# SAP/nested-hashing-psi

Measured on AMD Instinct MI355X. Metric: server PIE ciphertexts/sec, higher is better.
Workload: dtype u64

## Files before the change

### nested_hashing_psi_amd/csrc/kernels.hpp

```cpp
#pragma once
#include <hip/hip_runtime.h>

#include <atomic>
#include <vector>

#include "params.hpp"

namespace piehip {

struct PerDeviceOnce {
    std::atomic<unsigned long long> done{0};
    bool first_on_current_device()
    {
        int dev = 0;
        if (hipGetDevice(&dev) != hipSuccess || dev < 0 || dev > 63) return true;
        const unsigned long long bit = 1ULL << dev;
        return (done.fetch_or(bit) & bit) == 0;
    }
};

enum class NttKernel { radix2, blocked32, blocked16 };
struct NttRoute {
    NttKernel kernel;
    u32 s0;
    u32 global_stages;
    bool extra() const { return kernel != NttKernel::radix2 && !global_stages; }
};

struct NttPlan {
    const u64 *tables;
    const u64 *twp;
    const u64 *twc = nullptr;
    const u64 *twc_fold = nullptr;
    const u64 *twk16 = nullptr;
    const DevConsts *dc;
    u32 N, logN;
    u32 num_cus;
    u32 max_slots = 0;
    bool lane_order = false;
    bool fold = false;
    NttKernel lane_kernel = NttKernel::radix2;
    u32 lane_logn = 0;
    u32 lane_T = 0;
    u32 lane_kp = 16;
    bool small_moduli = false;
    bool xq_reuse = false;
    bool x_direct = false;
    bool fused_tensor = false;
    bool d01_eval_q = false;
    bool digits_with_d01 = false;
    bool digit_lift_lane = false;
    bool digit_lift_std = false;
    u32 transform_cus() const
    {
        if (!max_slots) return num_cus;
        const u32 c = (max_slots + 1) / 2;
        return c < num_cus ? (c ? c : 1u) : num_cus;
    }
};
void ntt_plan_decide(NttPlan &pl, bool lazy_ok, bool small_moduli);
NttRoute ntt_route(const NttPlan &pl, bool inverse, bool sigma, bool folded);

void build_twc_table(const u64 *nat_pairs, u32 logN, u32 s0, std::vector<u64> &out);
void build_twk16_table(const u64 *nat_pairs, u32 s0, u32 slice_log, std::vector<u64> &out);
void ntt_sigma_inverse_map(u32 logN, u32 s0, std::vector<u32> &map);
void ntt16_sigma_inverse_map(u32 logN, u32 s0, std::vector<u32> &map);
struct NttExtra {
    u64 *copy_out = nullptr;
    u32 copy_K = 1, copy_L = 1, copy_M = 1;
    u32 skip_L = 0, skip_M = 0;
    bool lazy_out = false;
    bool folded = false;
    bool x_lane_in = false;
};
void launch_ntt(const NttPlan &pl, u64 *data, u32 nlimbs, u32 mod_base, u32 mod_count, bool inverse, hipStream_t st,
                bool sigma = false, bool folded = false, const NttExtra *ex = nullptr);
void launch_ntt_fast(const NttPlan &pl, const u64 *twc, u32 s0, u64 *data, u32 nlimbs, u32 mod_base, u32 mod_count, bool inverse,
                     bool sigma, hipStream_t st, const u64 *lift_src = nullptr, u32 lift_L = 0, const NttExtra *ex = nullptr);
struct Ntt16Digits {
    const u64 *d2;
    size_t stride2;
    u64 *dig;
    u32 nb, L;
};
void launch_ntt16(const NttPlan &pl, u64 *data, u32 nlimbs, u32 mod_base, u32 mod_count, bool inverse, bool sigma, hipStream_t st,
                  const NttExtra *ex, const Ntt16Digits *dg = nullptr);
#ifndef PIEHIP_FUSE_TENSOR
#define PIEHIP_FUSE_TENSOR 1
#endif
#ifndef PIEHIP_D01_EVAL_Q
#define PIEHIP_D01_EVAL_Q 1
#endif
void launch_ntt16_tensor(const NttPlan &pl, const u64 *e, u64 *d, u32 nb, u32 M, hipStream_t st, u32 eval_q_L = 0);
void launch_ntt_digits(const NttPlan &pl, const u64 *d2, u64 *dig, u32 nb, u32 L, bool sigma, hipStream_t st);

struct StageAXOut {
    u64 *out = nullptr;
    u32 M = 0, logns = 0;
};
void launch_stage_a(const DevConsts *dc, u32 N, u32 L, u32 K, u32 b, u32 E, const u64 *idx, const u64 *minus,
                    const u64 *db, u64 *acc, hipStream_t st, bool small_moduli, u32 bstride = 0, u32 h0 = 0, u32 hn = 0, u32 nq = 1,
                    u32 q = 0, const StageAXOut *xo = nullptr);
static const u32 STAGE_A_MAX_QUERIES = 8;
struct StageAQueries {
    const u64 *idx[STAGE_A_MAX_QUERIES];
    const u64 *minus[STAGE_A_MAX_QUERIES];
};
void launch_stage_a_batch(const DevConsts *dc, u32 N, u32 L, u32 K, u32 b, u32 E, const StageAQueries &qs, u32 nq, const u64 *db,
                          u64 *acc, hipStream_t st, bool small_moduli, u32 bstride = 0, u32 h0 = 0, u32 hn = 0,
                          const StageAXOut *xo = nullptr);

void launch_expand_q_to_qp(const DevConsts *dc, u32 N, u32 L, const u64 *in, size_t in_stride_outer,
                           size_t in_stride_inner, u32 n_outer, u64 *out, u32 out_polys, u32 out_slot, hipStream_t st,
                           bool small_moduli, bool fold = false, bool skip_q = false);
void launch_scale_pq_expand(const DevConsts *dc, u32 N, u32 L, const u64 *in, size_t in_stride_outer,
                            size_t in_stride_inner, u32 n_outer, u64 *out, u32 out_polys, u32 out_slot, hipStream_t st,
                            bool small_moduli, bool fold = false);
void launch_expand_both(const DevConsts *dc, u32 N, u32 L, const u64 *x, size_t sx, const u64 *y, size_t sy, size_t si, u32 n_outer,
                        u64 *out, hipStream_t st, bool small_moduli, bool fold = false, bool skip_q = false);
void launch_tensor(const DevConsts *dc, u32 N, u32 M, const u64 *e, u64 *d, u32 nb, hipStream_t st, bool small_moduli);
void launch_scale_round(const DevConsts *dc, u32 N, u32 L, const u64 *d, u32 nb, u64 *out01, size_t stride01, u64 *out2,
                        size_t stride2, hipStream_t st, bool small_moduli, bool fold = false, bool fold_comp2 = false, bool p_only01 = false);
void launch_digits(const DevConsts *dc, u32 N, u32 L, const u64 *d2, size_t stride2, u32 nb, u64 *dig, hipStream_t st,
                   bool fold = false);
void launch_relin_mac(const DevConsts *dc, u32 N, u32 L, const u64 *d01, size_t stride01, const u64 *dig, const u64 *key,
                      const u64 *mask, u64 *out, u32 nb, hipStream_t st, bool small_moduli, const u32 *out_map = nullptr, size_t key_stride = 0,
                      u32 key_group = 1, u32 sigma_T = 0, u32 sigma_kp = 16, u32 mask_div = 1, const u64 *eqp = nullptr, u32 eqp_M = 0);
void launch_bcast_mul_plain(const DevConsts *dc, u32 N, u32 L, const u64 *x, size_t xs, u32 group, const u64 *pt, size_t ps_outer,
                            size_t ps_inner, u64 *out, u32 nct, hipStream_t st);
void launch_rot_prepare(const DevConsts *dc, u32 N, u32 L, const u64 *x, const u32 *maps, u32 map_group, bool acc, bool identity_first,
                        u64 *d01, u64 *d2, u32 nct, hipStream_t st);
void launch_sum_mul_plain(const DevConsts *dc, u32 N, u32 L, const u64 *x, u32 group, const u64 *pt, size_t pt_stride, u64 *out,
                          size_t out_stride, u32 ngroups, hipStream_t st);
void launch_host_flag(u64 *flag_dev, u64 value, hipStream_t st);
void launch_ct_add(const DevConsts *dc, u32 N, u32 L, const u64 *x, const u64 *y, u64 *out, u32 nct, hipStream_t st);
void launch_ct_mul_plain(const DevConsts *dc, u32 N, u32 L, const u64 *x, const u64 *pt, size_t pt_stride, u64 *out,
                         u32 nct, hipStream_t st, u32 pt_div = 1);
bool launch_limb_drop(const DevConsts *dc, u32 N, u32 L, u32 keep, const u64 *in, u64 *out, u32 npoly, hipStream_t st);
void launch_permute(u32 N, const u64 *in, const u32 *map, u64 *out, u32 nrows, hipStream_t st);
void launch_encode_scatter(const DevConsts *dc, u32 N, u32 M, const int64_t *slots, u32 B, const u32 *inv_pos, u64 *u,
                           u32 npt, hipStream_t st);
void launch_encode_lift(const DevConsts *dc, u32 N, u32 L, u32 M, const u64 *u, u64 *out, u32 npt, hipStream_t st, u32 l0 = 0);

void launch_stage_a_slice(const DevConsts *dc, u32 N, u32 L, u32 u_lo, u32 un, u32 b, u32 E, const StageAQueries &qs, u32 nq,
                          const u64 *db, u64 *acc, hipStream_t st, bool small_moduli);
void launch_place_accumulators(u32 N, u32 L, u32 K, u32 u_lo, u32 un, u32 bin_lo, u32 bn, u32 nq, const u64 *src, u64 *acc,
                               const StageAXOut *xo, hipStream_t st);

size_t hash_sort_temp_bytes(u32 n, u32 e);
hipError_t launch_hash_build(const u64 *d_tab, const u64 *d_items, u32 n, u32 k, u32 e, u32 K, u32 b, u32 E, u64 evict_seed,
                             u64 shuffle_seed, u64 *d_tbl, u32 *d_keys, u32 *d_vals, u32 *d_start, void *d_temp, size_t temp_bytes,
                             u32 *d_fail, hipStream_t st);
void launch_shuffle_rows(u64 *d_tbl, u32 rows, u32 b, u32 E, u64 seed, hipStream_t st);
void launch_gather_slots(const u64 *d_tbl, u32 B, u32 K, u32 b, u32 E, u64 t, int64_t *d_slots, u32 *d_fail, hipStream_t st);
void launch_mask_slots(u64 t, u32 b, u32 B, u64 seed, int64_t *d_out, hipStream_t st);

void launch_enc_message(const DevConsts *dc, u32 N, u32 L, u32 M, const u64 *coeff_t, const int32_t *e, u64 *em, u32 nct, hipStream_t st);
void launch_enc_finish(const DevConsts *dc, u32 N, u32 L, const u64 *em, const u64 *sk, const u64 *a_in, u64 *out, u32 nct,
                       hipStream_t st);
void launch_ks_finish(const DevConsts *dc, u32 N, u32 L, const u64 *e, const u64 *sk, const u64 *s_from, u64 *ks, hipStream_t st);
void launch_square(const DevConsts *dc, u32 N, u32 L, const u64 *s, u64 *s2, hipStream_t st);
void launch_dec_dot(const DevConsts *dc, u32 N, u32 L, const u64 *ct, const u64 *sk, u64 *xs, u32 nct, hipStream_t st);
void launch_dec_round(const DevConsts *dc, u32 N, u32 L, u32 M, const u64 *xs, u64 *coeff_t, u32 nct, hipStream_t st);
void launch_decode_gather(const DevConsts *dc, u32 N, u32 M, const u64 *u, const u32 *slot_pos, u32 B, int64_t *slots, u32 nct,
                          hipStream_t st);

struct SeedJob {
    u64 *dst;
    u32 seed[8];
};
static const u32 SEED_MAX_JOBS_PER_LAUNCH = 65535;
void launch_expand_uniform(const DevConsts *dc, u32 N, u32 L, const SeedJob *jobs, u32 njobs, hipStream_t st);

}
```

### nested_hashing_psi_amd/csrc/kernels_ntt.hip

```cpp
#include "kernels.hpp"

#include <algorithm>
#include <cassert>

namespace piehip {

static const u32 NTT_LDS_MAX_LOG = 14;

struct NttArgs {
    u64 *data;
    const u64 *tables;
    const DevConsts *dc;
    u32 N, logN;
    u32 s0;
    u32 mod_base, mod_count;
};

template <bool INV>
__global__ void __launch_bounds__(1024) ntt_lds_generic(NttArgs a)
{
    extern __shared__ u64 s[];
    const u32 tid = threadIdx.x, nthr = blockDim.x;
    const u32 nl = a.N >> a.s0;
    const u32 limb = blockIdx.x >> a.s0, blk = blockIdx.x & ((1u << a.s0) - 1);
    const u32 mod = a.mod_base + limb % a.mod_count;
    const Mod m = a.dc->mod[mod];
    const u64 q = m.q, q2 = 2 * m.q;
    const u64 *tw = a.tables + (size_t)mod * 4 * a.N + (INV ? 2 * (size_t)a.N : 0);
    const u64 *tws = tw + a.N;
    u64 *g = a.data + (size_t)limb * a.N + (size_t)blk * nl;

    for (u32 i = tid; i < nl; i += nthr) s[i] = g[i];
    __syncthreads();

    if (!INV) {
        u32 logt = a.logN - a.s0 - 1;
        for (u32 ml = 1; ml < nl; ml <<= 1, logt--) {
            const u32 t = 1u << logt;
            for (u32 bi = tid; bi < nl / 2; bi += nthr) {
                const u32 i = bi >> logt, j = bi & (t - 1);
                const u32 x = (i << (logt + 1)) + j;
                const u32 k = (ml << a.s0) + blk * ml + i;
                const u64 w = tw[k], ws = tws[k];
                u64 u = s[x];
                u = u >= q2 ? u - q2 : u;
                const u64 v = mul_shoup_lazy(s[x + t], w, ws, q);
                s[x] = u + v;
                s[x + t] = u - v + q2;
            }
            __syncthreads();
        }
        for (u32 i = tid; i < nl; i += nthr) {
            u64 v = s[i];
            v = v >= q2 ? v - q2 : v;
            g[i] = v >= q ? v - q : v;
        }
    } else {
        u32 logt = 0;
        for (u32 hl = nl >> 1; hl >= 1; hl >>= 1, logt++) {
            const u32 t = 1u << logt;
            for (u32 bi = tid; bi < nl / 2; bi += nthr) {
                const u32 i = bi >> logt, j = bi & (t - 1);
                const u32 x = (i << (logt + 1)) + j;
                const u32 k = (hl << a.s0) + blk * hl + i;
                const u64 w = tw[k], ws = tws[k];
                const u64 u = s[x], v = s[x + t];
                const u64 sm = u + v;
                s[x] = sm >= q2 ? sm - q2 : sm;
                s[x + t] = mul_shoup_lazy(u - v + q2, w, ws, q);
            }
            __syncthreads();
        }
        if (a.s0 == 0) {
            for (u32 i = tid; i < nl; i += nthr) g[i] = mul_shoup(s[i], m.n_inv, m.n_inv_sh, q);
        } else {
            for (u32 i = tid; i < nl; i += nthr) {
                u64 v = s[i];
                g[i] = v >= q ? v - q : v;
            }
        }
    }
}

template <bool INV>
__global__ void __launch_bounds__(256) ntt_global_stage(NttArgs a, u32 mstage, u32 last_inverse)
{
    const u32 half = a.N >> 1;
    const u32 bi = blockIdx.x * 256 + threadIdx.x;
    const u32 limb = blockIdx.y;
    if (bi >= half) return;
    const u32 mod = a.mod_base + limb % a.mod_count;
    const Mod m = a.dc->mod[mod];
    const u64 q = m.q;
    const u64 *tw = a.tables + (size_t)mod * 4 * a.N + (INV ? 2 * (size_t)a.N : 0);
    const u64 *tws = tw + a.N;
    u32 logm = 0;
    while ((1u << logm) < mstage) logm++;
    const u32 logt = a.logN - 1 - logm, t = 1u << logt;
    const u32 i = bi >> logt, j = bi & (t - 1);
    const size_t x = (size_t)limb * a.N + ((size_t)i << (logt + 1)) + j;
    const u64 w = tw[mstage + i], ws = tws[mstage + i];
    const u64 u = a.data[x], v = a.data[x + t];
    if (!INV) {
        const u64 p = mul_shoup(v, w, ws, q);
        a.data[x] = addmod(u, p, q);
        a.data[x + t] = submod(u, p, q);
    } else {
        u64 sm = addmod(u, v, q);
        u64 df = mul_shoup(submod(u, v, q), w, ws, q);
        if (last_inverse) {
            sm = mul_shoup(sm, m.n_inv, m.n_inv_sh, q);
            df = mul_shoup(df, m.n_inv, m.n_inv_sh, q);
        }
        a.data[x] = sm;
        a.data[x + t] = df;
    }
}

static PerDeviceOnce g_attr_set[2];

NttRoute ntt_route(const NttPlan &pl, bool inverse, bool sigma, bool folded)
{
    assert((!sigma || pl.lane_order) && (!folded || pl.fold));
    const u32 s0 = pl.logN > NTT_LDS_MAX_LOG ? pl.logN - NTT_LDS_MAX_LOG : 0;
    if (!pl.lane_order) return {NttKernel::radix2, s0, s0};
    if (pl.lane_kernel == NttKernel::blocked16 && folded == pl.fold && (inverse || sigma)) return {NttKernel::blocked16, folded ? 1u : 0u, 0};
    if (folded) return {NttKernel::blocked32, 1, 0};
    return {NttKernel::blocked32, s0, s0};
}

void ntt_plan_decide(NttPlan &pl, bool lazy_ok, bool small_moduli)
{
    pl.lane_order = lazy_ok && pl.logN >= 12;
    pl.small_moduli = small_moduli;
    if (!pl.lane_order) return;
    const bool k16 = pl.logN >= 13 && pl.logN <= 15;
    pl.lane_kernel = k16 ? NttKernel::blocked16 : NttKernel::blocked32;
    pl.fold = pl.logN == 14 || pl.logN == 15;
    pl.lane_logn = pl.logN - ntt_route(pl, true, true, pl.fold).s0;
    pl.lane_T = (1u << pl.lane_logn) / (k16 ? 16 : 32);
    pl.lane_kp = k16 ? 8 : 16;
    pl.xq_reuse = ntt_route(pl, true, false, pl.fold).extra();
    pl.fused_tensor = PIEHIP_FUSE_TENSOR && k16 && small_moduli;
    pl.d01_eval_q = PIEHIP_D01_EVAL_Q && pl.fused_tensor;
    pl.digits_with_d01 = k16 && small_moduli;
    pl.x_direct = pl.xq_reuse && k16 && small_moduli;
    const NttRoute std_fwd = ntt_route(pl, false, false, false);
    pl.digit_lift_std = std_fwd.kernel == NttKernel::blocked32 && std_fwd.s0 == 0;
    pl.digit_lift_lane = pl.digit_lift_std && !k16;
}

void launch_ntt_digits(const NttPlan &pl, const u64 *d2, u64 *dig, u32 nb, u32 L, bool sigma, hipStream_t st)
{
    assert(sigma ? pl.digit_lift_lane : pl.digit_lift_std);
    launch_ntt_fast(pl, pl.twc, 0, dig, nb * L * L, 0, L, false, sigma, st, d2, L);
}

void launch_ntt(const NttPlan &pl, u64 *data, u32 nlimbs, u32 mod_base, u32 mod_count, bool inverse, hipStream_t st, bool sigma,
                bool folded, const NttExtra *ex)
{
    if (!nlimbs) return;
    const NttRoute r = ntt_route(pl, inverse, sigma, folded);
    if (r.kernel == NttKernel::blocked16) {
        launch_ntt16(pl, data, nlimbs, mod_base, mod_count, inverse, sigma, st, ex);
        return;
    }
    if (folded) {
        NttExtra exf;
        if (ex) exf = *ex;
        exf.folded = true;
        launch_ntt_fast(pl, pl.twc_fold, 1, data, nlimbs, mod_base, mod_count, inverse, sigma, st, nullptr, 0, &exf);
        return;
    }
    NttArgs a;
    a.data = data;
    a.tables = pl.tables;
    a.dc = pl.dc;
    a.N = pl.N;
    a.logN = pl.logN;
    a.s0 = r.s0;
    a.mod_base = mod_base;
    a.mod_count = mod_count;
    const u32 nl = pl.N >> a.s0;
    const size_t lds = (size_t)nl * sizeof(u64);
    const u32 threads = std::min(std::max(nl / 2, 64u), 1024u);
    const bool radix2 = r.kernel == NttKernel::radix2;
    if (radix2 && g_attr_set[inverse ? 1 : 0].first_on_current_device())
        (void)hipFuncSetAttribute(inverse ? (const void *)ntt_lds_generic<true> : (const void *)ntt_lds_generic<false>,
                                  hipFuncAttributeMaxDynamicSharedMemorySize, (1 << NTT_LDS_MAX_LOG) * 8);
    const dim3 ggrid((pl.N / 2 + 255) / 256, nlimbs);
    if (!inverse) {
        for (u32 ms = 1; ms < (1u << r.global_stages); ms <<= 1)
            hipLaunchKernelGGL(ntt_global_stage<false>, ggrid, dim3(256), 0, st, a, ms, 0u);
        if (radix2) hipLaunchKernelGGL(ntt_lds_generic<false>, dim3(nlimbs << a.s0), dim3(threads), lds, st, a);
    } else if (radix2) {
        hipLaunchKernelGGL(ntt_lds_generic<true>, dim3(nlimbs << a.s0), dim3(threads), lds, st, a);
    }
    if (!radix2) launch_ntt_fast(pl, pl.twc, r.s0, data, nlimbs, mod_base, mod_count, inverse, sigma, st, nullptr, 0, ex);
    if (inverse)
        for (u32 ms = (1u << r.global_stages) >> 1; ms >= 1; ms >>= 1)
            hipLaunchKernelGGL(ntt_global_stage<true>, ggrid, dim3(256), 0, st, a, ms, ms == 1 ? 1u : 0u);
}

}
```

### nested_hashing_psi_amd/csrc/kernels_pie.hip

```cpp
#include <stdlib.h>

#include <cassert>

#include <algorithm>

#include "kernels.hpp"
#include "madasm.h"
#include "stage_a_common.h"

namespace piehip {

static const u32 TPB = 256;

typedef u64 u64x2 __attribute__((ext_vector_type(2)));


template <int BPT>
__global__ void __launch_bounds__(TPB) stage_a_kernel(const DevConsts *__restrict__ dc, u32 N, u32 L, u32 K, u32 b, u32 E,
                                                      const u64 *__restrict__ idx, const u64 *__restrict__ minus,
                                                      const u64 *__restrict__ db, u64 *__restrict__ acc, u32 bstride, u32 h0,
                                                      u32 nq, u32 q)
{
    const u32 n = 2 * (blockIdx.x * TPB + threadIdx.x);
    const u32 l = blockIdx.y;
    const u32 groups = b / BPT;
    const u32 h = h0 + blockIdx.z / groups, beta0 = (blockIdx.z % groups) * BPT;
    if (n >= N) return;
    const Mod m = dc->mod[l];
    const size_t LN = (size_t)L * N;
    const u64 *pi = idx + ((size_t)h * E) * 2 * LN + (size_t)l * N + n;
    const u64 *pd = db + (((size_t)h * bstride + beta0) * E) * LN + (size_t)l * N + n;
    const size_t bin_stride = (size_t)E * LN;
    U128 a[BPT][2][2];
#pragma unroll
    for (int t = 0; t < BPT; t++)
#pragma unroll
        for (int c = 0; c < 2; c++) a[t][c][0] = a[t][c][1] = U128{0, 0};
    for (u32 j = 0; j < E; j++) {
        const u64x2 i0 = *reinterpret_cast<const u64x2 *>(pi + (size_t)j * 2 * LN);
        const u64x2 i1 = *reinterpret_cast<const u64x2 *>(pi + (size_t)j * 2 * LN + LN);
        u64x2 d[BPT];
#pragma unroll
        for (int t = 0; t < BPT; t++) {
            typedef u64 u64v2 __attribute__((ext_vector_type(2)));
            const u64v2 v = __builtin_nontemporal_load(reinterpret_cast<const u64v2 *>(pd + (size_t)t * bin_stride + (size_t)j * LN));
            d[t].x = v.x, d[t].y = v.y;
        }
#pragma unroll
        for (int t = 0; t < BPT; t++) {
            mac128(a[t][0][0], i0.x, d[t].x);
            mac128(a[t][0][1], i0.y, d[t].y);
            mac128(a[t][1][0], i1.x, d[t].x);
            mac128(a[t][1][1], i1.y, d[t].y);
        }
        if ((j & 31) == 31) {
#pragma unroll
            for (int t = 0; t < BPT; t++)
#pragma unroll
                for (int c = 0; c < 2; c++)
#pragma unroll
                    for (int e = 0; e < 2; e++) a[t][c][e] = U128{reduce128(a[t][c][e], m), 0};
        }
    }
    const u64x2 m0 = *reinterpret_cast<const u64x2 *>(minus + (size_t)l * N + n);
    const u64x2 m1 = *reinterpret_cast<const u64x2 *>(minus + LN + (size_t)l * N + n);
#pragma unroll
    for (int t = 0; t < BPT; t++) {
        u64 *po = acc + ((((size_t)(beta0 + t) * nq + q) * K + h) * 2) * LN + (size_t)l * N + n;
        u64x2 r0, r1;
        r0.x = addmod(reduce128(a[t][0][0], m), m0.x, m.q);
        r0.y = addmod(reduce128(a[t][0][1], m), m0.y, m.q);
        r1.x = addmod(reduce128(a[t][1][0], m), m1.x, m.q);
        r1.y = addmod(reduce128(a[t][1][1], m), m1.y, m.q);
        *reinterpret_cast<u64x2 *>(po) = r0;
        *reinterpret_cast<u64x2 *>(po + LN) = r1;
    }
}

static const int SA_DEPTH = 4;
template <int BPT>
__global__ void __launch_bounds__(TPB) stage_a_mad_kernel(const DevConsts *__restrict__ dc, u32 N, u32 L, u32 K, u32 b, u32 E,
                                                          const u64 *__restrict__ idx, const u64 *__restrict__ minus,
                                                          const u64 *__restrict__ db, u64 *__restrict__ acc, u32 bstride, u32 h0,
                                                          u32 nq, u32 q, StageAXOut xo)
{
    const u32 nl = threadIdx.x;
    const u32 n = blockIdx.x * TPB + nl;
    const u32 l = blockIdx.y;
    const u32 groups = b / BPT;
    const u32 h = h0 + blockIdx.z / groups, beta0 = (blockIdx.z % groups) * BPT;
    if (n >= N) return;
    const Mod m = dc->mod[l];
    const size_t LN = (size_t)L * N;
    const u64 *pi = idx + ((size_t)h * E) * 2 * LN + (size_t)l * N + blockIdx.x * TPB;
    const u64 *pd = db + (((size_t)h * bstride + beta0) * E) * LN + (size_t)l * N + blockIdx.x * TPB;
    const size_t bin_stride = (size_t)E * LN;
    ColAcc a[BPT][2];
#pragma unroll
    for (int t = 0; t < BPT; t++) a[t][0] = a[t][1] = ColAcc{0, 0, 0};
    auto load_term = [&](u32 j, u64 (&vi)[2], u64 (&vd)[BPT]) {
        const u64 *pij = pi + (size_t)j * 2 * LN, *pdj = pd + (size_t)j * LN;
        vi[0] = pij[nl];
        vi[1] = (pij + LN)[nl];
#pragma unroll
        for (int t = 0; t < BPT; t++) vd[t] = __builtin_nontemporal_load(pdj + (size_t)t * bin_stride + nl);
    };
    u64 qiv[SA_DEPTH][2], qdv[SA_DEPTH][BPT];
#pragma unroll
    for (int d = 0; d < SA_DEPTH; d++)
        if ((u32)d < E) load_term(d, qiv[d], qdv[d]);
    auto term = [&](u32 j, u64 (&vi)[2], u64 (&vd)[BPT]) {
        const Split30 i0 = split30(vi[0]), i1 = split30(vi[1]);
#pragma unroll
        for (int t = 0; t < BPT; t++) colacc_mac2(a[t][0], a[t][1], i0, i1, vd[t]);
        if (j + SA_DEPTH < E) load_term(j + SA_DEPTH, vi, vd);
        if ((j % COLACC_MAX_TERMS) == COLACC_MAX_TERMS - 1 && j + 1 < E) {
#pragma unroll
            for (int t = 0; t < BPT; t++) colacc_carry(a[t][0]), colacc_carry(a[t][1]);
        }
        if ((j % COLACC_MAX_TOTAL) == COLACC_MAX_TOTAL - 1 && j + 1 < E) {
#pragma unroll
            for (int t = 0; t < BPT; t++)
#pragma unroll
                for (int c = 0; c < 2; c++) {
                    const u64 r = reduce124(colacc_value(a[t][c]), m);
                    a[t][c] = ColAcc{r & 0x3FFFFFFFull, r >> 30, 0};
                }
        }
    };
    for (u32 j = 0; j < E; j += SA_DEPTH) {
#pragma unroll
        for (int d = 0; d < SA_DEPTH; d++)
            if (j + d < E) term(j + d, qiv[d], qdv[d]);
    }
    const bool xdir = h == 0 && xo.out != nullptr;
    const u32 noff = n + ((xdir ? ~0u : 0u) & (lane_home(n, xo.logns) - n));
#pragma unroll
    for (int t = 0; t < BPT; t++) {
        const size_t row = (size_t)(beta0 + t) * nq + q;
        u64 *const base = xdir ? xo.out + ((row * 4) * xo.M + l) * N : acc + ((row * K + h) * 2) * LN + (size_t)l * N;
        const size_t cstride = xdir ? (size_t)xo.M * N : LN;
        u64 *const po = base + noff;
#pragma unroll
        for (int c = 0; c < 2; c++)
            po[(size_t)c * cstride] = addmod_nb(colacc_reduce<true>(a[t][c], m, 0 - m.q), minus[(size_t)c * LN + (size_t)l * N + n], m.q);
    }
}

template <int BPT, int Q, int DEPTH>
__global__ void __launch_bounds__(TPB) stage_a_mad_batch_kernel(const DevConsts *__restrict__ dc, u32 N, u32 L, u32 K, u32 b, u32 E,
                                                                StageAQueries qs, const u64 *__restrict__ db, u64 *__restrict__ acc,
                                                                u32 bstride, u32 h0, u32 nq, u32 q0, u32 tiles, StageAXOut xo)
{
    StageATile tl;
    if (!stage_a_tile((N + TPB - 1) / TPB, L, tiles, (b + BPT - 1) / BPT, tl)) return;
    const u32 nl = threadIdx.x, n0 = tl.bx * TPB, l = tl.l, h = h0 + tl.hz, beta0 = tl.grp * BPT;
    const u32 n = n0 + nl;
    if (n >= N) return;
    const u32 tmax = __builtin_amdgcn_readfirstlane(min((u32)BPT, b - beta0) - 1);
    const Mod m = dc->mod[l];
    const size_t LN = (size_t)L * N;
    const size_t ioff = ((size_t)h * E) * 2 * LN + (size_t)l * N + n0;
    const u64 *pd = db + (((size_t)h * bstride + beta0) * E) * LN + (size_t)l * N + n0;
    const size_t bin_stride = (size_t)E * LN;
    ColAcc a[Q][BPT][2];
#pragma unroll
    for (int q = 0; q < Q; q++)
#pragma unroll
        for (int t = 0; t < BPT; t++) a[q][t][0] = a[q][t][1] = ColAcc{0, 0, 0};
    auto load_term = [&](u32 j, u64 (&vi)[Q][2], u64 (&vd)[BPT]) {
#pragma unroll
        for (int q = 0; q < Q; q++) {
            const u64 *pij = qs.idx[q] + ioff + (size_t)j * 2 * LN;
            vi[q][0] = pij[nl];
            vi[q][1] = (pij + LN)[nl];
        }
        const u64 *pdj = pd + (size_t)j * LN;
#pragma unroll
        for (int t = 0; t < BPT; t++) vd[t] = __builtin_nontemporal_load(pdj + (size_t)min((u32)t, tmax) * bin_stride + nl);
    };
    u64 qiv[DEPTH][Q][2], qdv[DEPTH][BPT];
#pragma unroll
    for (int d = 0; d < DEPTH; d++)
        if ((u32)d < E) load_term(d, qiv[d], qdv[d]);
    auto term = [&](u32 j, u64 (&vi)[Q][2], u64 (&vd)[BPT]) {
#pragma unroll
        for (int q = 0; q < Q; q++) {
            const Split30 i0 = split30(vi[q][0]), i1 = split30(vi[q][1]);
#pragma unroll
            for (int t = 0; t < BPT; t++) colacc_mac2(a[q][t][0], a[q][t][1], i0, i1, vd[t]);
        }
        if (j + DEPTH < E) load_term(j + DEPTH, vi, vd);
        if ((j % COLACC_MAX_TERMS) == COLACC_MAX_TERMS - 1 && j + 1 < E) {
#pragma unroll
            for (int q = 0; q < Q; q++)
#pragma unroll
                for (int t = 0; t < BPT; t++) colacc_carry(a[q][t][0]), colacc_carry(a[q][t][1]);
        }
        if ((j % COLACC_MAX_TOTAL) == COLACC_MAX_TOTAL - 1 && j + 1 < E) {
#pragma unroll
            for (int q = 0; q < Q; q++)
#pragma unroll
                for (int t = 0; t < BPT; t++)
#pragma unroll
                    for (int c = 0; c < 2; c++) {
                        const u64 r = colacc_reduce<true>(a[q][t][c], m, 0 - m.q);
                        a[q][t][c] = ColAcc{r & 0x3FFFFFFFull, r >> 30, 0};
                    }
        }
    };
    for (u32 j = 0; j < E; j += DEPTH) {
#pragma unroll
        for (int d = 0; d < DEPTH; d++)
            if (j + d < E) term(j + d, qiv[d], qdv[d]);
    }
    const bool xdir = h == 0 && xo.out != nullptr;
    const u32 noff = n + ((xdir ? ~0u : 0u) & (lane_home(n, xo.logns) - n));
#pragma unroll
    for (int q = 0; q < Q; q++) {
        u64 mi[2];
#pragma unroll
        for (int c = 0; c < 2; c++) mi[c] = qs.minus[q][(size_t)c * LN + (size_t)l * N + n];
#pragma unroll
        for (int t = 0; t < BPT; t++) {
            if ((u32)t > tmax) continue;
            const size_t row = (size_t)(beta0 + t) * nq + q0 + q;
            u64 *const base = xdir ? xo.out + ((row * 4) * xo.M + l) * N : acc + ((row * K + h) * 2) * LN + (size_t)l * N;
            const size_t cstride = xdir ? (size_t)xo.M * N : LN;
            u64 *const po = base + noff;
#pragma unroll
            for (int c = 0; c < 2; c++) po[(size_t)c * cstride] = addmod_nb(colacc_reduce<true>(a[q][t][c], m, 0 - m.q), mi[c], m.q);
        }
    }
}

static void launch_stage_a_uniform(const DevConsts *dc, u32 N, u32 L, u32 K, u32 b, u32 E, const u64 *idx, const u64 *minus,
                                   const u64 *db, u64 *acc, hipStream_t st, bool mad, u32 bstride, u32 h0, u32 hn, int bpt, u32 nq,
                                   u32 q, StageAXOut xo)
{
    const int cpt = mad ? 1 : 2;
    dim3 grid((N / cpt + TPB - 1) / TPB, L, hn * (b / bpt));
#define SA(B_)                                                                                                       \
    do {                                                                                                             \
        if (mad) hipLaunchKernelGGL(stage_a_mad_kernel<B_>, grid, dim3(TPB), 0, st, dc, N, L, K, b, E, idx, minus, db, acc, bstride, h0, nq, q, xo); \
        else hipLaunchKernelGGL(stage_a_kernel<B_>, grid, dim3(TPB), 0, st, dc, N, L, K, b, E, idx, minus, db, acc, bstride, h0, nq, q);  \
    } while (0)
    switch (bpt) {
        case 8: hipLaunchKernelGGL(stage_a_kernel<8>, grid, dim3(TPB), 0, st, dc, N, L, K, b, E, idx, minus, db, acc, bstride, h0, nq, q); break;
        case 7: SA(7); break;
        case 6: SA(6); break;
        case 5: SA(5); break;
        case 4: SA(4); break;
        case 3: SA(3); break;
        case 2: SA(2); break;
        default: SA(1); break;
    }
#undef SA
}

void launch_stage_a(const DevConsts *dc, u32 N, u32 L, u32 K, u32 b, u32 E, const u64 *idx, const u64 *minus,
                    const u64 *db, u64 *acc, hipStream_t st, bool small_moduli, u32 bstride, u32 h0, u32 hn, u32 nq, u32 q,
                    const StageAXOut *xop)
{
    StageAXOut xo;
    if (xop && small_moduli) xo = *xop;
    if (!bstride) bstride = b;
    if (!hn) hn = K - h0;
    if (!nq) nq = 1;
    const bool mad = small_moduli;
    const u32 cap = mad ? 7 : 8;
    u32 bpt = 0;
    for (u32 c = cap; c >= 4; c--)
        if (b % c == 0) {
            bpt = c;
            break;
        }
    if (b <= cap) bpt = b;
    const size_t LN = (size_t)L * N;
    if (bpt) {
        launch_stage_a_uniform(dc, N, L, K, b, E, idx, minus, db, acc, st, mad, bstride, h0, hn, (int)bpt, nq, q, xo);
        return;
    }
    const u32 full = (b / cap) * cap, rest = b - full;
    launch_stage_a_uniform(dc, N, L, K, full, E, idx, minus, db, acc, st, mad, bstride, h0, hn, (int)cap, nq, q, xo);
    StageAXOut xr = xo;
    if (xr.out) xr.out += (size_t)full * nq * 4 * xr.M * N;
    launch_stage_a_uniform(dc, N, L, K, rest, E, idx, minus, db + (size_t)full * E * LN, acc + (size_t)full * nq * K * 2 * LN, st, mad,
                           bstride, h0, hn, (int)rest, nq, q, xr);
}

template <int Q, int BPT>
static void launch_stage_a_batch_qb(const DevConsts *dc, u32 N, u32 L, u32 K, u32 nb, u32 E, const StageAQueries &qs, const u64 *db,
                                    u64 *acc, hipStream_t st, u32 bstride, u32 h0, u32 hn, u32 nq, u32 q0, StageAXOut xo)
{
    const u32 nx = (N + TPB - 1) / TPB;
    constexpr int DEPTH = (Q == 4 || Q * BPT >= 9) ? 2 : 3;
    hipLaunchKernelGGL((stage_a_mad_batch_kernel<BPT, Q, DEPTH>), stage_a_grid(nx, L, hn, (nb + BPT - 1) / BPT), dim3(TPB), 0, st, dc, N, L, K,
                       nb, E, qs, db, acc, bstride, h0, nq, q0, nx * L * hn, xo);
}
template <int Q>
static void launch_stage_a_batch_q(const DevConsts *dc, u32 N, u32 L, u32 K, u32 b, u32 E, const StageAQueries &qs, const u64 *db,
                                   u64 *acc, hipStream_t st, u32 bstride, u32 h0, u32 hn, u32 nq, u32 q0, StageAXOut xo)
{
    constexpr u32 cap = Q == 2 ? 4 : 3;
    u32 bpt = 1, best = ~0u;
    for (u32 g = 1; g <= cap && g <= b; g++) {
        const u32 loads = ((b + g - 1) / g) * (2 * Q + g);
        if (loads <= best) best = loads, bpt = g;
    }
    if constexpr (cap >= 4)
        if (bpt == 4) return launch_stage_a_batch_qb<Q, 4>(dc, N, L, K, b, E, qs, db, acc, st, bstride, h0, hn, nq, q0, xo);
    if constexpr (cap >= 3)
        if (bpt == 3) return launch_stage_a_batch_qb<Q, 3>(dc, N, L, K, b, E, qs, db, acc, st, bstride, h0, hn, nq, q0, xo);
    if (bpt == 2) return launch_stage_a_batch_qb<Q, 2>(dc, N, L, K, b, E, qs, db, acc, st, bstride, h0, hn, nq, q0, xo);
    return launch_stage_a_batch_qb<Q, 1>(dc, N, L, K, b, E, qs, db, acc, st, bstride, h0, hn, nq, q0, xo);
}
void launch_stage_a_batch(const DevConsts *dc, u32 N, u32 L, u32 K, u32 b, u32 E, const StageAQueries &qs, u32 nq, const u64 *db,
                          u64 *acc, hipStream_t st, bool small_moduli, u32 bstride, u32 h0, u32 hn, const StageAXOut *xop)
{
    StageAXOut xo;
    if (xop && small_moduli) xo = *xop;
    if (!bstride) bstride = b;
    if (!hn) hn = K - h0;
    u32 q0 = 0;
    while (small_moduli && nq - q0 >= 2) {
        const u32 left = nq - q0, g = left == 5 || left == 6 ? 3 : std::min(left, 4u);
        StageAQueries sub = {};
        for (u32 q = 0; q < g; q++) sub.idx[q] = qs.idx[q0 + q], sub.minus[q] = qs.minus[q0 + q];
        if (g == 2) launch_stage_a_batch_q<2>(dc, N, L, K, b, E, sub, db, acc, st, bstride, h0, hn, nq, q0, xo);
        else if (g == 3) launch_stage_a_batch_q<3>(dc, N, L, K, b, E, sub, db, acc, st, bstride, h0, hn, nq, q0, xo);
        else launch_stage_a_batch_q<4>(dc, N, L, K, b, E, sub, db, acc, st, bstride, h0, hn, nq, q0, xo);
        q0 += g;
    }
    for (; q0 < nq; q0++)
        launch_stage_a(dc, N, L, K, b, E, qs.idx[q0], qs.minus[q0], db, acc, st, small_moduli, bstride, h0, hn, nq, q0, xop);
}

#define PIE_ITER_FENCE() __builtin_amdgcn_sched_barrier(0)
typedef const __attribute__((address_space(4))) DevConsts *DcC;
__device__ __forceinline__ DcC dc_iter(const DevConsts *dc)
{
    u64 v = (u64)dc;
    asm volatile("" : "+s"(v));
    return (DcC)v;
}
__device__ __forceinline__ Mod ld_mod(DcC c, u32 i)
{
    Mod m;
    m.q = c->mod[i].q, m.r0 = c->mod[i].r0, m.r1 = c->mod[i].r1, m.n_inv = 0, m.n_inv_sh = 0;
    m.fconst = c->mod[i].fconst, m.fshift = c->mod[i].fshift, m.pad = 0;
    return m;
}

__device__ __forceinline__ u64 neg_u(u64 m)
{
    u64 n = 0 - m;
    asm("" : "+s"(n));
    return n;
}
__device__ __forceinline__ u64 sel_neg(u64 x, u64 t, u32 &mask)
{
    u32 lo, hi, k;
    asm("v_ashrrev_i32 %[k], 31, %[th]\n\t"
        "v_bfi_b32 %[lo], %[k], %[xl], %[tl]\n\t"
        "v_bfi_b32 %[hi], %[k], %[xh], %[th]"
        : [lo] "=&v"(lo), [hi] "=&v"(hi), [k] "=&v"(k)
        : [xl] "v"((u32)x), [xh] "v"((u32)(x >> 32)), [tl] "v"((u32)t), [th] "v"((u32)(t >> 32)));
    mask = k;
    return ((u64)hi << 32) | lo;
}
__device__ __forceinline__ u64 csub_u(u64 x, u64 negm)
{
    u32 k;
    return sel_neg(x, x + negm, k);
}
__device__ __forceinline__ u64 mul_shoup_lazy_u(u64 a, u64 w, u64 wsh, u64 q) { return a * w - mulhi(a, wsh) * q; }
__device__ __forceinline__ u64 mul_shoup_u(u64 a, u64 w, u64 wsh, u64 q, u64 negq) { return csub_u(mul_shoup_lazy_u(a, w, wsh, q), negq); }
__device__ __forceinline__ u64 fixfrac_u(u64 y, const Mod &m) { return mulhi(y << m.fshift, m.fconst) >> 3; }
__device__ __forceinline__ void divmod_shoup_u(u64 a, u64 w, u64 wsh, u64 q, u64 negq, u64 &quot, u64 &rem)
{
    const u64 qe = mulhi(a, wsh);
    const u64 r = a * w - qe * q;
    u32 k;
    rem = sel_neg(r, r + negq, k);
    quot = qe + 1 + (u64)(int64_t)(int32_t)k;
}
__device__ __forceinline__ u64 reduce123_u(U128 z, const Mod &m, u64 negq, u64 neg2q)
{
    const u64 mu = (m.r1 << 59) | (m.r0 >> 5);
    const u64 zh = (z.hi << 5) | (z.lo >> 59);
    const u64 qhat = mulhi(zh, mu);
    return csub_u(csub_u(z.lo - qhat * m.q, neg2q), negq);
}

#define PIE_SHOUP63_HEAD                                        \
    "v_mad_u64_u32 v[60:61], vcc, %[al], %[sh], 0\n\t"          \
    "v_mad_u64_u32 v[64:65], vcc, %[al], %[wl], 0\n\t"          \
    "v_mad_u64_u32 v[60:61], vcc, %[ah], %[sl], v[60:61]\n\t"   \
    "v_mad_u64_u32 v[66:67], vcc, %[al], %[wh], 0\n\t"          \
    "v_lshlrev_b32 v70, 1, %[ah]\n\t"                           \
    "v_mad_u64_u32 v[66:67], vcc, %[ah], %[wl], v[66:67]\n\t"   \
    "v_lshrrev_b64 v[60:61], 31, v[60:61]\n\t"                  \
    "v_mad_u64_u32 v[62:63], vcc, v70, %[sh], v[60:61]\n\t"     \
    "v_mad_u64_u32 v[66:67], vcc, v62, %[nqh], v[66:67]\n\t"    \
    "v_mad_u64_u32 v[66:67], vcc, v63, %[nql], v[66:67]\n\t"    \
    "v_add_u32 v65, v65, v66\n\t"
#define PIE_SHOUP63_IN(a, w, wsh, nq)                                                                                        \
    [al] "v"((u32)(a)), [ah] "v"((u32)((a) >> 32)), [wl] "s"((u32)(w)), [wh] "s"((u32)((w) >> 32)), [sl] "s"((u32)((wsh) >> 1)), \
        [sh] "s"((u32)((wsh) >> 33)), [nql] "s"((u32)(nq)), [nqh] "s"((u32)((nq) >> 32))
__device__ __forceinline__ u64 shoup63_lazy(u64 a, u64 w, u64 wsh, u64 nq)
{
    u64 r;
    asm(PIE_SHOUP63_HEAD
        "v_mad_u64_u32 %[r], vcc, v62, %[nql], v[64:65]"
        : [r] "=v"(r)
        : PIE_SHOUP63_IN(a, w, wsh, nq)
        : PIE_ASM_CLOB);
    return r;
}
__device__ __forceinline__ u64 shoup63(u64 a, u64 w, u64 wsh, u64 nq)
{
    u32 lo, hi;
    const u64 n2q = 2 * nq;
    asm(PIE_SHOUP63_HEAD
        "v_mad_u64_u32 v[64:65], vcc, v62, %[nql], v[64:65]\n\t"
        "v_lshl_add_u64 v[68:69], v[64:65], 0, %[n2q]\n\t"
        "v_ashrrev_i32 v71, 31, v69\n\t"
        "v_bfi_b32 v64, v71, v64, v68\n\t"
        "v_bfi_b32 v65, v71, v65, v69\n\t"
        "v_lshl_add_u64 v[68:69], v[64:65], 0, %[n1q]\n\t"
        "v_ashrrev_i32 v71, 31, v69\n\t"
        "v_bfi_b32 %[lo], v71, v64, v68\n\t"
        "v_bfi_b32 %[hi], v71, v65, v69"
        : [lo] "=v"(lo), [hi] "=v"(hi)
        : PIE_SHOUP63_IN(a, w, wsh, nq), [n2q] "s"(n2q), [n1q] "s"(nq)
        : PIE_ASM_CLOB);
    return ((u64)hi << 32) | lo;
}
__device__ __forceinline__ void divmod63(u64 a, u64 w, u64 wsh, u64 nq, u64 &quot, u64 &rem)
{
    u32 lo, hi;
    u64 qt;
    const u64 n2q = 2 * nq;
    asm(PIE_SHOUP63_HEAD
        "v_mad_u64_u32 v[64:65], vcc, v62, %[nql], v[64:65]\n\t"
        "v_lshl_add_u64 v[68:69], v[64:65], 0, %[n2q]\n\t"
        "v_ashrrev_i64 v[60:61], 63, v[68:69]\n\t"
        "v_bfi_b32 v64, v60, v64, v68\n\t"
        "v_bfi_b32 v65, v60, v65, v69\n\t"
        "v_lshl_add_u64 v[62:63], v[60:61], 1, v[62:63]\n\t"
        "v_lshl_add_u64 v[68:69], v[64:65], 0, %[n1q]\n\t"
        "v_ashrrev_i64 v[60:61], 63, v[68:69]\n\t"
        "v_bfi_b32 %[lo], v60, v64, v68\n\t"
        "v_bfi_b32 %[hi], v60, v65, v69\n\t"
        "v_lshl_add_u64 v[62:63], v[60:61], 0, v[62:63]\n\t"
        "v_lshl_add_u64 %[qt], v[62:63], 0, 3"
        : [lo] "=v"(lo), [hi] "=v"(hi), [qt] "=v"(qt)
        : PIE_SHOUP63_IN(a, w, wsh, nq), [n2q] "s"(n2q), [n1q] "s"(nq)
        : PIE_ASM_CLOB);
    quot = qt;
    rem = ((u64)hi << 32) | lo;
}
__device__ __forceinline__ u64 mulhi_sb(u64 a, u64 b)
{
    u64 r;
    asm("v_mul_hi_u32 v60, %[al], %[bl]\n\t"
        "v_mov_b32 v61, 0\n\t"
        "v_mad_u64_u32 v[62:63], vcc, %[al], %[bh], v[60:61]\n\t"
        "v_mad_u64_u32 v[62:63], vcc, %[ah], %[bl], v[62:63]\n\t"
        "v_mad_u64_u32 v[66:67], s[96:97], %[ah], %[bh], 0\n\t"
        "v_lshrrev_b64 v[64:65], 32, v[62:63]\n\t"
        "v_addc_co_u32 v65, vcc, 0, v65, vcc\n\t"
        "v_lshl_add_u64 %[r], v[66:67], 0, v[64:65]"
        : [r] "=v"(r)
        : [al] "v"((u32)a), [ah] "v"((u32)(a >> 32)), [bl] "s"((u32)b), [bh] "s"((u32)(b >> 32))
        : PIE_ASM_CLOB, "s96", "s97");
    return r;
}
__device__ __forceinline__ void colacc_mac_small(ColAcc &a, u32 v, u64 c)
{
    const Split30 s = split30(c);
    a.c0 = mad_u(v, s.lo, a.c0);
    a.c1 = mad_u(v, s.hi, a.c1);
}

template <bool ASM>
__device__ __forceinline__ u64 mshoup(u64 a, u64 w, u64 wsh, u64 q, u64 negq)
{
    return ASM ? shoup63(a, w, wsh, negq) : mul_shoup_u(a, w, wsh, q, negq);
}
template <bool ASM>
__device__ __forceinline__ void mdivmod(u64 a, u64 w, u64 wsh, u64 q, u64 negq, u64 &quot, u64 &rem)
{
    if (ASM)
        divmod63(a, w, wsh, negq, quot, rem);
    else
        divmod_shoup_u(a, w, wsh, q, negq, quot, rem);
}
template <bool ASM>
__device__ __forceinline__ u64 mfixfrac(u64 y, const Mod &m)
{
    return ASM ? (mulhi_sb(y << m.fshift, m.fconst) >> 3) : fixfrac_u(y, m);
}

template <u32 NS, bool MAD>
__device__ __forceinline__ U128 dot128(const u64 *y, const u64 (&c)[NS])
{
    if (MAD) {
        ColAcc a = {0, 0, 0};
#pragma unroll
        for (u32 i = 0; i < NS; i++) colacc_mac(a, split30(y[i]), split30(c[i]));
        return colacc_value(a);
    }
    U128 acc = {0, 0};
#pragma unroll
    for (u32 i = 0; i < NS; i++) mac128(acc, y[i], c[i]);
    return acc;
}

template <u32 NS, bool MAD, bool LZ = false>
__device__ __forceinline__ u64 crt_out(const u64 *y, const u64 (&hat)[NS], u64 v, u64 prodmod, const Mod &tm, u64 negq, u64 neg2q)
{
    if (MAD && NS <= 7) {
        ColAcc a = {0, 0, 0};
#pragma unroll
        for (u32 i = 0; i < NS; i++) colacc_mac(a, split30(y[i]), split30(hat[i]));
        colacc_mac_small(a, (u32)v, tm.q - prodmod);
        return LZ ? colacc_reduce123_lazy(a, tm, negq) : colacc_reduce<false>(a, tm, negq);
    }
    U128 acc = dot128<NS, MAD>(y, hat);
    mac128(acc, v, tm.q - prodmod);
    return reduce128(acc, tm);
}

__device__ __forceinline__ void fold_load(const DevConsts *dc, u32 a, u64 u, u64 v, u64 &x0, u64 &x1)
{
    PIE_ITER_FENCE();
    const DcC c = dc_iter(dc);
    const u64 q = c->mod[a].q, nq = neg_u(q);
    x0 = shoup63(u + v, c->fold_ia[a], c->fold_ia_sh[a], nq);
    x1 = shoup63(u + (4 * q - v), c->fold_ib[a], c->fold_ib_sh[a], nq);
}
__device__ __forceinline__ void fold_store(const DevConsts *dc, u32 a, u64 u, u64 v, u64 &y0, u64 &y1)
{
    const DcC c = dc_iter(dc);
    const u64 q = c->mod[a].q;
    const u64 t = shoup63_lazy(v, c->fold_w[a], c->fold_w_sh[a], neg_u(q));
    y0 = u + t;
    y1 = u + (4 * q - t);
}

template <u32 L, bool MAD, bool YIN, int NP, bool LZ = false>
__device__ __forceinline__ void expand_core(const DevConsts *dc, const u64 (&x)[NP][L], u64 (&out)[NP][2 * L + 1])
{
    constexpr u32 Lp = L + 1;
    u64 y[NP][L];
    u64 fsum[NP];
#pragma unroll
    for (int p = 0; p < NP; p++) fsum[p] = 0;
#pragma unroll
    for (u32 i = 0; i < L; i++) {
        PIE_ITER_FENCE();
        const DcC c = dc_iter(dc);
        const Mod mi = ld_mod(c, i);
        const u64 w = c->qhat_inv[i], wsh = c->qhat_inv_sh[i], nq = neg_u(mi.q);
#pragma unroll
        for (int p = 0; p < NP; p++) {
            out[p][i] = x[p][i];
            y[p][i] = YIN ? x[p][i] : mshoup<MAD>(x[p][i], w, wsh, mi.q, nq);
            fsum[p] += mfixfrac<MAD>(y[p][i], mi);
        }
    }
#pragma unroll
    for (u32 j = 0; j < Lp; j++) {
        PIE_ITER_FENCE();
        const DcC c = dc_iter(dc);
        const Mod pj = ld_mod(c, L + j);
        u64 hat[L];
#pragma unroll
        for (u32 i = 0; i < L; i++) hat[i] = c->qhat_modp[i][j];
        const u64 prodmod = c->Q_modp[j], nq = neg_u(pj.q), n2q = neg_u(2 * pj.q);
#pragma unroll
        for (int p = 0; p < NP; p++) out[p][L + j] = crt_out<L, MAD, LZ>(y[p], hat, (fsum[p] + FIX_HALF) >> 60, prodmod, pj, nq, n2q);
    }
}

template <u32 L, bool MAD, bool YIN, int NP, bool LZ = false>
__device__ __forceinline__ void scale_pq_core(const DevConsts *dc, const u64 (&x)[NP][L], u64 (&out)[NP][2 * L + 1])
{
    constexpr u32 Lp = L + 1;
    u64 y[NP][L];
    u64 fsum[NP];
    U128 itot[NP];
#pragma unroll
    for (int p = 0; p < NP; p++) fsum[p] = 0, itot[p] = U128{0, 0};
#pragma unroll
    for (u32 i = 0; i < L; i++) {
        PIE_ITER_FENCE();
        const DcC c = dc_iter(dc);
        const Mod mi = ld_mod(c, i);
        const u64 w = c->qhat_inv[i], wsh = c->qhat_inv_sh[i], pw = c->P_modq[i], pwsh = c->P_modq_sh[i], nq = neg_u(mi.q);
#pragma unroll
        for (int p = 0; p < NP; p++) {
            y[p][i] = YIN ? x[p][i] : mshoup<MAD>(x[p][i], w, wsh, mi.q, nq);
            u64 fl, z;
            mdivmod<MAD>(y[p][i], pw, pwsh, mi.q, nq, fl, z);
            add128(itot[p], U128{fl, 0});
            fsum[p] += mfixfrac<MAD>(z, mi);
        }
    }
    u64 yp[NP][Lp];
    u64 fs2[NP];
#pragma unroll
    for (int p = 0; p < NP; p++) {
        add128(itot[p], U128{(fsum[p] + FIX_HALF) >> 60, 0});
        fs2[p] = 0;
    }
#pragma unroll
    for (u32 j = 0; j < Lp; j++) {
        PIE_ITER_FENCE();
        const DcC c = dc_iter(dc);
        const Mod pj = ld_mod(c, L + j);
        u64 col[L];
#pragma unroll
        for (u32 i = 0; i < L; i++) col[i] = c->PI_modp[i][j];
        const u64 w = c->phat_inv[j], wsh = c->phat_inv_sh[j], nq = neg_u(pj.q);
#pragma unroll
        for (int p = 0; p < NP; p++) {
            u64 r;
            if (MAD) {
                ColAcc a = {itot[p].lo, 0, 0};
#pragma unroll
                for (u32 i = 0; i < L; i++) colacc_mac(a, split30(y[p][i]), split30(col[i]));
                r = LZ ? colacc_reduce123_lazy(a, pj, nq) : colacc_reduce<false>(a, pj, nq);
            } else {
                U128 acc = dot128<L, MAD>(y[p], col);
                add128(acc, itot[p]);
                r = reduce128(acc, pj);
            }
            out[p][L + j] = r;
            yp[p][j] = mshoup<MAD>(r, w, wsh, pj.q, nq);
            fs2[p] += mfixfrac<MAD>(yp[p][j], pj);
        }
    }
#pragma unroll
    for (u32 i = 0; i < L; i++) {
        PIE_ITER_FENCE();
        const DcC c = dc_iter(dc);
        const Mod mi = ld_mod(c, i);
        u64 hat[Lp];
#pragma unroll
        for (u32 j = 0; j < Lp; j++) hat[j] = c->phat_modq[j][i];
        const u64 prodmod = c->P_modq[i], nq = neg_u(mi.q), n2q = neg_u(2 * mi.q);
#pragma unroll
        for (int p = 0; p < NP; p++) out[p][i] = crt_out<Lp, MAD, LZ>(yp[p], hat, (fs2[p] + FIX_HALF) >> 60, prodmod, mi, nq, n2q);
    }
}

template <bool SCALE, bool FOLD, u32 L, bool MAD, bool SKIPQ>
__device__ __forceinline__ void expand_body(const DevConsts *__restrict__ dc, u32 N, const u64 *__restrict__ in, size_t so, size_t si,
                                            u64 *__restrict__ out, u32 out_polys, u32 out_slot, u32 by)
{
    constexpr bool YIN = FOLD && (SCALE || SKIPQ);
    const u32 n = blockIdx.x * TPB + threadIdx.x;
    const u32 H = N / 2;
    if (n >= (FOLD ? H : N)) return;
    const u32 o = by >> 1, c = by & 1;
    constexpr u32 M = 2 * L + 1;
    const u64 *pin = in + (size_t)o * so + (size_t)c * si + n;
    u64 *pout = out + ((size_t)(o * out_polys + out_slot + c) * M) * N + n;
    constexpr int NP = FOLD ? 2 : 1;
    u64 x[NP][L], y[NP][M];
#pragma unroll
    for (u32 i = 0; i < L; i++) {
        if (YIN) {
            PIE_ITER_FENCE();
            const DcC c = dc_iter(dc);
            const u64 q = c->mod[i].q, nq = neg_u(q), u = pin[(size_t)i * N], v = pin[(size_t)i * N + H];
            x[0][i] = shoup63(u + v, c->fold_iaq[i], c->fold_iaq_sh[i], nq);
            x[NP - 1][i] = shoup63(u + (4 * q - v), c->fold_ibq[i], c->fold_ibq_sh[i], nq);
        } else if (FOLD) {
            fold_load(dc, i, pin[(size_t)i * N], pin[(size_t)i * N + H], x[0][i], x[NP - 1][i]);
        } else {
            x[0][i] = pin[(size_t)i * N];
        }
    }
    constexpr bool LZ = FOLD && MAD;
    if (SCALE)
        scale_pq_core<L, MAD, YIN, NP, LZ>(dc, x, y);
    else
        expand_core<L, MAD, YIN, NP, LZ>(dc, x, y);
#pragma unroll
    for (u32 a = 0; a < M; a++) {
        if (!SCALE && a < L && SKIPQ) continue;
        PIE_ITER_FENCE();
        if (FOLD) {
            u64 y0, y1;
            fold_store(dc, a, y[0][a], y[NP - 1][a], y0, y1);
            pout[(size_t)a * N] = y0;
            pout[(size_t)a * N + H] = y1;
        } else {
            pout[(size_t)a * N] = y[0][a];
        }
    }
}

template <bool SCALE, bool FOLD, u32 L, bool MAD, bool SKIPQ>
__global__ void __launch_bounds__(TPB) expand_kernel(const DevConsts *__restrict__ dc, u32 N, const u64 *__restrict__ in,
                                                     size_t so, size_t si, u64 *__restrict__ out, u32 out_polys, u32 out_slot)
{
    expand_body<SCALE, FOLD, L, MAD, SKIPQ>(dc, N, in, so, si, out, out_polys, out_slot, blockIdx.y);
}
template <bool FOLD, u32 L, bool MAD, bool SKIPQ>
__global__ void __launch_bounds__(TPB) expand_both_kernel(const DevConsts *__restrict__ dc, u32 N, const u64 *__restrict__ x, size_t sx,
                                                          const u64 *__restrict__ y, size_t sy, size_t si, u64 *__restrict__ out,
                                                          u32 n_outer)
{
    if (blockIdx.y < 2 * n_outer)
        expand_body<true, FOLD, L, MAD, false>(dc, N, y, sy, si, out, 4, 2, blockIdx.y);
    else
        expand_body<false, FOLD, L, MAD, SKIPQ>(dc, N, x, sx, si, out, 4, 0, blockIdx.y - 2 * n_outer);
}
void launch_expand_both(const DevConsts *dc, u32 N, u32 L, const u64 *x, size_t sx, const u64 *y, size_t sy, size_t si, u32 n_outer,
                        u64 *out, hipStream_t st, bool small_moduli, bool fold, bool skip_q)
{
    dim3 grid(((fold ? N / 2 : N) + TPB - 1) / TPB, n_outer * 4);
#define EB(F_, L_, M_, Q_) hipLaunchKernelGGL((expand_both_kernel<F_, L_, M_, Q_>), grid, dim3(TPB), 0, st, dc, N, x, sx, y, sy, si, out, n_outer)
#define EBL(L_)                                                                          \
    case L_:                                                                             \
        if (fold && small_moduli) { if (skip_q) EB(true, L_, true, true); else EB(true, L_, true, false); }      \
        else if (fold) { if (skip_q) EB(true, L_, false, true); else EB(true, L_, false, false); }                 \
        else if (small_moduli) { if (skip_q) EB(false, L_, true, true); else EB(false, L_, true, false); }       \
        else { if (skip_q) EB(false, L_, false, true); else EB(false, L_, false, false); }                         \
        break;
    switch (L) { EBL(1) EBL(2) EBL(3) EBL(4) EBL(5) EBL(6) EBL(7) }
#undef EBL
#undef EB
}

static void launch_expand_common(bool scale, bool fold, const DevConsts *dc, u32 N, u32 L, const u64 *in, size_t so, size_t si,
                                 u32 n_outer, u64 *out, u32 out_polys, u32 out_slot, hipStream_t st, bool small_moduli, bool skip_q = false)
{
    dim3 grid(((fold ? N / 2 : N) + TPB - 1) / TPB, n_outer * 2);
#define EX(S_, F_, L_, Q_)                                                                                                    \
    do {                                                                                                                      \
        if (small_moduli)                                                                                                   \
            hipLaunchKernelGGL((expand_kernel<S_, F_, L_, true, Q_>), grid, dim3(TPB), 0, st, dc, N, in, so, si, out, out_polys, out_slot); \
        else                                                                                                                  \
            hipLaunchKernelGGL((expand_kernel<S_, F_, L_, false, Q_>), grid, dim3(TPB), 0, st, dc, N, in, so, si, out, out_polys, out_slot); \
    } while (0)
#define EXL(L_)                                                         \
    case L_:                                                            \
        if (scale) {                                                    \
            if (fold) EX(true, true, L_, false); else EX(true, false, L_, false); \
        } else if (skip_q) {                                            \
            if (fold) EX(false, true, L_, true); else EX(false, false, L_, true); \
        } else {                                                        \
            if (fold) EX(false, true, L_, false); else EX(false, false, L_, false); \
        }                                                               \
        break;
    switch (L) { EXL(1) EXL(2) EXL(3) EXL(4) EXL(5) EXL(6) EXL(7) }
#undef EXL
#undef EX
}
void launch_expand_q_to_qp(const DevConsts *dc, u32 N, u32 L, const u64 *in, size_t so, size_t si, u32 n_outer, u64 *out,
                           u32 out_polys, u32 out_slot, hipStream_t st, bool small_moduli, bool fold, bool skip_q)
{
    launch_expand_common(false, fold, dc, N, L, in, so, si, n_outer, out, out_polys, out_slot, st, small_moduli, skip_q);
}
void launch_scale_pq_expand(const DevConsts *dc, u32 N, u32 L, const u64 *in, size_t so, size_t si, u32 n_outer, u64 *out,
                            u32 out_polys, u32 out_slot, hipStream_t st, bool small_moduli, bool fold)
{
    launch_expand_common(true, fold, dc, N, L, in, so, si, n_outer, out, out_polys, out_slot, st, small_moduli);
}

template <bool MAD>
__global__ void __launch_bounds__(TPB) tensor_kernel(const DevConsts *dc, u32 N, u32 M, const u64 *__restrict__ e,
                                                     u64 *__restrict__ d)
{
    const u32 n = 2 * (blockIdx.x * TPB + threadIdx.x);
    if (n >= N) return;
    const u32 a = blockIdx.y, bin = blockIdx.z;
    const Mod m = dc->mod[a];
    const size_t MN = (size_t)M * N;
    const u64 *pe = e + (size_t)bin * 4 * MN + (size_t)a * N + n;
    u64 *pd = d + (size_t)bin * 3 * MN + (size_t)a * N + n;
    const u64x2 va0 = *reinterpret_cast<const u64x2 *>(pe), va1 = *reinterpret_cast<const u64x2 *>(pe + MN),
                vb0 = *reinterpret_cast<const u64x2 *>(pe + 2 * MN), vb1 = *reinterpret_cast<const u64x2 *>(pe + 3 * MN);
    u64x2 r0, r1, r2;
#pragma unroll
    for (int k = 0; k < 2; k++) {
        u64 a0 = k ? va0.y : va0.x, a1 = k ? va1.y : va1.x, b0 = k ? vb0.y : vb0.x, b1 = k ? vb1.y : vb1.x;
        u64 d0, d1, d2;
        if (MAD) {
            const u64 nq = neg_u(m.q), n2q = neg_u(2 * m.q), n4q = neg_u(4 * m.q);
            a0 = csub_u(csub_u(a0, n4q), n2q), a1 = csub_u(csub_u(a1, n4q), n2q);
            b0 = csub_u(csub_u(b0, n4q), n2q), b1 = csub_u(csub_u(b1, n4q), n2q);
            const Split30 sa0 = split30(a0), sa1 = split30(a1), sb0 = split30(b0), sb1 = split30(b1);
            ColAcc c = {0, 0, 0};
            colacc_mac(c, sa0, sb0);
            d0 = colacc_reduce<false>(c, m, nq);
            c = ColAcc{0, 0, 0};
            colacc_mac(c, sa0, sb1);
            colacc_mac(c, sa1, sb0);
            d1 = colacc_reduce<false>(c, m, nq);
            c = ColAcc{0, 0, 0};
            colacc_mac(c, sa1, sb1);
            d2 = colacc_reduce<false>(c, m, nq);
        } else {
            d0 = mulmod(a0, b0, m);
            U128 x = mul128(a0, b1);
            mac128(x, a1, b0);
            d1 = reduce128(x, m);
            d2 = mulmod(a1, b1, m);
        }
        if (k) r0.y = d0, r1.y = d1, r2.y = d2;
        else r0.x = d0, r1.x = d1, r2.x = d2;
    }
    *reinterpret_cast<u64x2 *>(pd) = r0;
    *reinterpret_cast<u64x2 *>(pd + MN) = r1;
    *reinterpret_cast<u64x2 *>(pd + 2 * MN) = r2;
}
void launch_tensor(const DevConsts *dc, u32 N, u32 M, const u64 *e, u64 *d, u32 nb, hipStream_t st, bool small_moduli)
{
    dim3 grid((N / 2 + TPB - 1) / TPB, M, nb);
    if (small_moduli)
        hipLaunchKernelGGL(tensor_kernel<true>, grid, dim3(TPB), 0, st, dc, N, M, e, d);
    else
        hipLaunchKernelGGL(tensor_kernel<false>, grid, dim3(TPB), 0, st, dc, N, M, e, d);
}

template <u32 L, bool MAD, int NP, bool PRE = false, bool PONLY = false>
__device__ __forceinline__ void scale_round_core(const DevConsts *dc, const u64 (&d)[NP][2 * L + 1], u64 (&out)[NP][L], bool lz = false)
{
    constexpr u32 Lp = L + 1;
    u64 yp[NP][Lp];
    u64 fsum[NP];
    U128 itot[NP];
#pragma unroll
    for (int p = 0; p < NP; p++) fsum[p] = 0, itot[p] = U128{0, 0};
#pragma unroll
    for (u32 j = 0; j < Lp; j++) {
        PIE_ITER_FENCE();
        const DcC c = dc_iter(dc);
        const Mod pj = ld_mod(c, L + j);
        const u64 w = c->qp_hat_inv[L + j], wsh = c->qp_hat_inv_sh[L + j], tw = c->tQ_modp[j], twsh = c->tQ_modp_sh[j], nq = neg_u(pj.q);
#pragma unroll
        for (int p = 0; p < NP; p++) {
            yp[p][j] = PRE ? d[p][L + j] : mshoup<MAD>(d[p][L + j], w, wsh, pj.q, nq);
            u64 fl, z;
            mdivmod<MAD>(yp[p][j], tw, twsh, pj.q, nq, fl, z);
            add128(itot[p], U128{fl, 0});
            fsum[p] += mfixfrac<MAD>(z, pj);
        }
    }
#pragma unroll
    for (int p = 0; p < NP; p++) add128(itot[p], U128{(fsum[p] + FIX_HALF) >> 60, 0});
#pragma unroll
    for (u32 k = 0; k < L; k++) {
        PIE_ITER_FENCE();
        const DcC c = dc_iter(dc);
        const Mod qk = ld_mod(c, k);
        u64 col[Lp];
#pragma unroll
        for (u32 j = 0; j < Lp; j++) col[j] = c->tQF_modq[j][k];
        const u64 tp = c->tPinv_modq[k], nq = neg_u(qk.q);
#pragma unroll
        for (int p = 0; p < NP; p++) {
            if (MAD && L <= 6) {
                ColAcc a = {itot[p].lo, 0, 0};
#pragma unroll
                for (u32 j = 0; j < Lp; j++) colacc_mac(a, split30(yp[p][j]), split30(col[j]));
                if (PONLY)
                    ;
                else if (PRE)
                    a.c0 += d[p][k];
                else
                    colacc_mac(a, split30(d[p][k]), split30(tp));
                out[p][k] = (L <= 5 && lz) ? colacc_reduce123_lazy(a, qk, nq) : colacc_reduce<(L > 5)>(a, qk, nq);
            } else {
                U128 acc = dot128<Lp, MAD>(yp[p], col);
                if (PONLY)
                    ;
                else if (PRE)
                    add128(acc, U128{d[p][k], 0});
                else
                    mac128(acc, d[p][k], tp);
                add128(acc, itot[p]);
                out[p][k] = reduce128(acc, qk);
            }
        }
    }
}

template <bool FOLD, u32 L, bool MAD, bool PONLY>
__device__ __forceinline__ void scale_round_comp(const DevConsts *__restrict__ dc, u32 N, u32 n, const u64 *__restrict__ pin,
                                                 u64 *__restrict__ pout, bool fold_out, bool lz)
{
    const u32 H = N / 2;
    constexpr u32 M = 2 * L + 1;
    constexpr int NP = FOLD ? 2 : 1;
    u64 x[NP][M], y[NP][L];
#pragma unroll
    for (u32 a = PONLY ? L : 0; a < M; a++) {
        if (FOLD) {
            PIE_ITER_FENCE();
            const DcC c = dc_iter(dc);
            const u32 ak = a < L ? a : 0, aj = a < L ? 0 : a - L;
            const u64 q = c->mod[a].q, nq = neg_u(q), u = pin[(size_t)a * N], v = pin[(size_t)a * N + H];
            const u64 wa = a < L ? c->fold_iat[ak] : c->fold_iap[aj], was = a < L ? c->fold_iat_sh[ak] : c->fold_iap_sh[aj];
            const u64 wb = a < L ? c->fold_ibt[ak] : c->fold_ibp[aj], wbs = a < L ? c->fold_ibt_sh[ak] : c->fold_ibp_sh[aj];
            x[0][a] = shoup63(u + v, wa, was, nq);
            x[NP - 1][a] = shoup63(u + (4 * q - v), wb, wbs, nq);
        } else {
            x[0][a] = pin[(size_t)a * N];
        }
    }
    scale_round_core<L, MAD, NP, FOLD, PONLY>(dc, x, y, lz);
#pragma unroll
    for (u32 k = 0; k < L; k++) {
        PIE_ITER_FENCE();
        if (FOLD) {
            u64 y0 = y[0][k], y1 = y[NP - 1][k];
            if (fold_out) fold_store(dc, k, y[0][k], y[NP - 1][k], y0, y1);
            pout[(size_t)k * N] = y0;
            pout[(size_t)k * N + H] = y1;
        } else {
            pout[(size_t)k * N] = y[0][k];
        }
    }
}
template <bool FOLD, u32 L, bool MAD, bool P01 = false>
__global__ void __launch_bounds__(TPB) scale_round_kernel(const DevConsts *__restrict__ dc, u32 N, const u64 *__restrict__ d,
                                                          u64 *__restrict__ out01, size_t stride01,
                                                          u64 *__restrict__ out2, size_t stride2, u32 fold_comp2)
{
    const u32 n = blockIdx.x * TPB + threadIdx.x;
    if (n >= (FOLD ? N / 2 : N)) return;
    const u32 comp = blockIdx.y, bin = blockIdx.z;
    constexpr u32 M = 2 * L + 1;
    const u64 *pin = d + ((size_t)(bin * 3 + comp) * M) * N + n;
    u64 *pout = comp < 2 ? out01 + (size_t)bin * stride01 + (size_t)comp * L * N + n : out2 + (size_t)bin * stride2 + n;
    const bool lz = FOLD && MAD && comp < 2 && !fold_comp2;
    if (P01 && comp < 2)
        scale_round_comp<FOLD, L, MAD, true>(dc, N, n, pin, pout, true, lz);
    else
        scale_round_comp<FOLD, L, MAD, false>(dc, N, n, pin, pout, comp < 2 || fold_comp2, lz);
}
void launch_scale_round(const DevConsts *dc, u32 N, u32 L, const u64 *d, u32 nb, u64 *out01, size_t stride01, u64 *out2,
                        size_t stride2, hipStream_t st, bool small_moduli, bool fold, bool fold_comp2, bool p_only01)
{
    assert(!p_only01 || (small_moduli && !fold_comp2));
    dim3 grid(((fold ? N / 2 : N) + TPB - 1) / TPB, 3, nb);
#define SRK(F_, L_, M_, P_) \
    hipLaunchKernelGGL((scale_round_kernel<F_, L_, M_, P_>), grid, dim3(TPB), 0, st, dc, N, d, out01, stride01, out2, stride2, (fold_comp2 && F_) ? 1u : 0u)
#define SRL(L_)                                                                        \
    case L_:                                                                           \
        if (p_only01) {                                                                \
            if (fold) SRK(true, L_, true, true); else SRK(false, L_, true, true);      \
        } else if (small_moduli) {                                                     \
            if (fold) SRK(true, L_, true, false); else SRK(false, L_, true, false);    \
        } else {                                                                       \
            if (fold) SRK(true, L_, false, false); else SRK(false, L_, false, false);  \
        }                                                                              \
        break;
    switch (L) { SRL(1) SRL(2) SRL(3) SRL(4) SRL(5) SRL(6) SRL(7) }
#undef SRK
#undef SRL
}

__device__ __forceinline__ u64 digit_lift(const DevConsts *dc, u32 i, u32 j, u64 v)
{
    const Mod &mj = dc->mod[j];
    const u64 qi = dc->mod[i].q;
    u64 r = (qi < 2 * mj.q) ? (v >= mj.q ? v - mj.q : v) : barrett128(0, v, mj);
    if (v > qi / 2) r = submod(r, dc->qi_modqj[i][j], mj.q);
    return r;
}
template <bool FOLD>
__global__ void __launch_bounds__(TPB) digits_kernel(const DevConsts *__restrict__ dc, u32 N, u32 L, const u64 *__restrict__ d2,
                                                     size_t stride2, u64 *__restrict__ dig)
{
    const u32 n = blockIdx.x * TPB + threadIdx.x;
    const u32 H = N / 2;
    if (n >= (FOLD ? H : N)) return;
    const u32 i = blockIdx.y / L, j = blockIdx.y % L, bin = blockIdx.z;
    const u64 *pin = d2 + (size_t)bin * stride2 + (size_t)i * N + n;
    u64 *pout = dig + (((size_t)bin * L + i) * L + j) * N + n;
    if (FOLD) {
        u64 y0, y1;
        fold_store(dc, j, digit_lift(dc, i, j, pin[0]), digit_lift(dc, i, j, pin[H]), y0, y1);
        pout[0] = y0;
        pout[H] = y1;
    } else {
        pout[0] = digit_lift(dc, i, j, pin[0]);
    }
}
void launch_digits(const DevConsts *dc, u32 N, u32 L, const u64 *d2, size_t stride2, u32 nb, u64 *dig, hipStream_t st, bool fold)
{
    dim3 grid(((fold ? N / 2 : N) + TPB - 1) / TPB, L * L, nb);
    if (fold)
        hipLaunchKernelGGL(digits_kernel<true>, grid, dim3(TPB), 0, st, dc, N, L, d2, stride2, dig);
    else
        hipLaunchKernelGGL(digits_kernel<false>, grid, dim3(TPB), 0, st, dc, N, L, d2, stride2, dig);
}

template <bool MAD, int KP, int RPT = 1, bool EQ = false>
__global__ void __launch_bounds__(TPB) relin_mac_kernel(const DevConsts *__restrict__ dc, u32 N, u32 L, const u64 *__restrict__ d01,
                                                        size_t stride01, const u64 *__restrict__ dig,
                                                        const u64 *__restrict__ key0, const u64 *__restrict__ mask,
                                                        u64 *__restrict__ out, const u32 *__restrict__ out_map,
                                                        size_t key_stride, u32 key_group, u32 T, u32 mask_div, u32 nb,
                                                        const u64 *__restrict__ eqp, u32 eqp_M)
{
    static_assert(RPT == 1 || MAD, "two rows per thread: the column-accumulator path");
    static_assert(!EQ || MAD, "the own-limb term: the column-accumulator path");
    constexpr bool TILE = KP > 0;
    constexpr u32 TT = TILE ? TPB / (KP ? KP : 1) : 1;
    __shared__ u64x2 s_tile[TILE ? 2 * RPT : 1][TILE ? TPB : 1];
    u32 n = 2 * (blockIdx.x * TPB + threadIdx.x);
    u32 std_pair = 0;
    if (TILE) {
        const u32 tiles = T / TT, slice = blockIdx.x / tiles, tau0 = (blockIdx.x % tiles) * TT;
        const u32 k = threadIdx.x / TT, tt = threadIdx.x % TT;
        n = 2 * (slice * KP * T + k * T + tau0 + tt);
        std_pair = slice * KP * T + KP * tau0;
    }
    if (n >= N) return;
    const u32 j = blockIdx.y;
    u32 rows[RPT];
    bool has[RPT];
    if (RPT == 1) {
        rows[0] = blockIdx.z, has[0] = true;
    } else {
        const u32 k = blockIdx.z / key_group, q = blockIdx.z % key_group;
        rows[0] = 2 * k * key_group + q, has[0] = rows[0] < nb;
        rows[RPT - 1] = rows[0] + key_group, has[RPT - 1] = rows[RPT - 1] < nb;
        if (!has[0]) return;
    }
    const u32 bin = rows[0];
    const u64 *key = key0 + (size_t)(bin % key_group) * key_stride;
    const Mod m = dc->mod[j];
    const size_t LN = (size_t)L * N;
    const u32 po = TILE ? 0 : (out_map ? out_map[n] : n);
    u64x2 res[RPT][2];
    if (MAD) {
        ColAcc a[RPT][2][2];
#pragma unroll
        for (int r = 0; r < RPT; r++)
#pragma unroll
            for (int c = 0; c < 2; c++) a[r][c][0] = a[r][c][1] = ColAcc{0, 0, 0};
        for (u32 i = 0; i < L; i++) {
            const u64x2 k0 = *reinterpret_cast<const u64x2 *>(key + (((size_t)i * 2 + 0) * L + j) * N + n);
            const u64x2 k1 = *reinterpret_cast<const u64x2 *>(key + (((size_t)i * 2 + 1) * L + j) * N + n);
            const Split30 k0x = split30(k0.x), k0y = split30(k0.y), k1x = split30(k1.x), k1y = split30(k1.y);
#pragma unroll
            for (int r = 0; r < RPT; r++) {
                if (r && !has[r]) continue;
                const u64x2 d = *reinterpret_cast<const u64x2 *>(dig + (((size_t)rows[r] * L + i) * L + j) * N + n);
                const Split30 dx = split30(d.x), dy = split30(d.y);
                colacc_mac(a[r][0][0], dx, k0x);
                colacc_mac(a[r][0][1], dy, k0y);
                colacc_mac(a[r][1][0], dx, k1x);
                colacc_mac(a[r][1][1], dy, k1y);
            }
        }
        const u64 nq = 0 - m.q;
        if (EQ) {
            const u64 n2q = neg_u(2 * m.q), n4q = neg_u(4 * m.q);
            const u64 tp = dc->tPinv_modq[j], tpsh = dc->tPinv_modq_sh[j];
            const size_t MN = (size_t)eqp_M * N;
#pragma unroll
            for (int r = 0; r < RPT; r++) {
                if (r && !has[r]) continue;
                const u64 *pe = eqp + (size_t)rows[r] * 4 * MN + (size_t)j * N + n;
                const u64x2 va0 = *reinterpret_cast<const u64x2 *>(pe), va1 = *reinterpret_cast<const u64x2 *>(pe + MN),
                            vb0 = *reinterpret_cast<const u64x2 *>(pe + 2 * MN), vb1 = *reinterpret_cast<const u64x2 *>(pe + 3 * MN);
#pragma unroll
                for (int k = 0; k < 2; k++) {
                    const Split30 sa0 = split30(csub_u(csub_u(k ? va0.y : va0.x, n4q), n2q)), sa1 = split30(csub_u(csub_u(k ? va1.y : va1.x, n4q), n2q));
                    const Split30 sb0 = split30(csub_u(csub_u(k ? vb0.y : vb0.x, n4q), n2q)), sb1 = split30(csub_u(csub_u(k ? vb1.y : vb1.x, n4q), n2q));
                    ColAcc t = {0, 0, 0};
                    colacc_mac(t, sa0, sb0);
                    const u64 v0 = shoup63_lazy(colacc_reduce123_lazy(t, m, nq), tp, tpsh, nq);
                    t = ColAcc{0, 0, 0};
                    colacc_mac(t, sa0, sb1);
                    colacc_mac(t, sa1, sb0);
                    const u64 v1 = shoup63_lazy(colacc_reduce123_lazy(t, m, nq), tp, tpsh, nq);
                    a[r][0][k].c0 += v0 & 0x3FFFFFFFull, a[r][0][k].c1 += v0 >> 30;
                    a[r][1][k].c0 += v1 & 0x3FFFFFFFull, a[r][1][k].c1 += v1 >> 30;
                }
            }
        }
#pragma unroll
        for (int r = 0; r < RPT; r++) {
            if (r && !has[r]) continue;
            u64x2 mk;
            if (mask) mk = *reinterpret_cast<const u64x2 *>(mask + (size_t)(rows[r] / mask_div) * LN + (size_t)j * N + n);
#pragma unroll
            for (int c = 0; c < 2; c++) {
                const u64x2 s = *reinterpret_cast<const u64x2 *>(d01 + (size_t)rows[r] * stride01 + (size_t)c * LN + (size_t)j * N + n);
                a[r][c][0].c0 += s.x;
                a[r][c][1].c0 += s.y;
                res[r][c].x = colacc_reduce<false>(a[r][c][0], m, nq);
                res[r][c].y = colacc_reduce<false>(a[r][c][1], m, nq);
                if (mask) {
                    ColAcc p0 = {0, 0, 0}, p1 = {0, 0, 0};
                    colacc_mac(p0, split30(res[r][c].x), split30(mk.x));
                    colacc_mac(p1, split30(res[r][c].y), split30(mk.y));
                    res[r][c].x = colacc_reduce<false>(p0, m, nq);
                    res[r][c].y = colacc_reduce<false>(p1, m, nq);
                }
            }
        }
    } else {
        u64x2 mk;
        if (mask) mk = *reinterpret_cast<const u64x2 *>(mask + (size_t)(bin / mask_div) * LN + (size_t)j * N + n);
        U128 acc[2][2];
#pragma unroll
        for (int c = 0; c < 2; c++)
#pragma unroll
            for (int e = 0; e < 2; e++) acc[c][e] = U128{0, 0};
        for (u32 i = 0; i < L; i++) {
            const u64x2 d = *reinterpret_cast<const u64x2 *>(dig + (((size_t)bin * L + i) * L + j) * N + n);
            const u64x2 k0 = *reinterpret_cast<const u64x2 *>(key + (((size_t)i * 2 + 0) * L + j) * N + n);
            const u64x2 k1 = *reinterpret_cast<const u64x2 *>(key + (((size_t)i * 2 + 1) * L + j) * N + n);
            mac128(acc[0][0], d.x, k0.x);
            mac128(acc[0][1], d.y, k0.y);
            mac128(acc[1][0], d.x, k1.x);
            mac128(acc[1][1], d.y, k1.y);
        }
#pragma unroll
        for (int c = 0; c < 2; c++) {
            const u64x2 s = *reinterpret_cast<const u64x2 *>(d01 + (size_t)bin * stride01 + (size_t)c * LN + (size_t)j * N + n);
            add128(acc[c][0], U128{s.x, 0});
            add128(acc[c][1], U128{s.y, 0});
            res[0][c].x = reduce128(acc[c][0], m);
            res[0][c].y = reduce128(acc[c][1], m);
            if (mask) {
                res[0][c].x = mulmod(res[0][c].x, mk.x, m);
                res[0][c].y = mulmod(res[0][c].y, mk.y, m);
            }
        }
    }
#pragma unroll
    for (int r = 0; r < RPT; r++)
#pragma unroll
        for (int c = 0; c < 2; c++) {
            if (r && !has[r]) continue;
            const u64x2 v = res[r][c];
            if (TILE)
                s_tile[2 * r + c][KP * (threadIdx.x % TT) + threadIdx.x / TT] = v;
            else
                *reinterpret_cast<u64x2 *>(out + ((size_t)rows[r] * 2 + c) * LN + (size_t)j * N + po) = v;
        }
    if (TILE) {
        __syncthreads();
#pragma unroll
        for (int r = 0; r < RPT; r++)
#pragma unroll
            for (int c = 0; c < 2; c++) {
                if (r && !has[r]) continue;
                *reinterpret_cast<u64x2 *>(out + ((size_t)rows[r] * 2 + c) * LN + (size_t)j * N + 2 * (std_pair + threadIdx.x)) = s_tile[2 * r + c][threadIdx.x];
            }
    }
}
void launch_relin_mac(const DevConsts *dc, u32 N, u32 L, const u64 *d01, size_t stride01, const u64 *dig, const u64 *key,
                      const u64 *mask, u64 *out, u32 nb, hipStream_t st, bool small_moduli, const u32 *out_map, size_t key_stride,
                      u32 key_group, u32 sigma_T, u32 sigma_kp, u32 mask_div, const u64 *eqp, u32 eqp_M)
{
    assert(!eqp || (small_moduli && eqp_M >= L));
    if (!key_group) key_group = 1;
    if (!mask_div) mask_div = 1;
    const bool tile = out_map && (sigma_kp == 16 || sigma_kp == 8) && sigma_T >= TPB / sigma_kp && sigma_T % (TPB / sigma_kp) == 0 &&
                      (N / 2) % TPB == 0;
    const int kp = tile ? (int)sigma_kp : 0;
    const bool two = small_moduli && nb >= 2 * key_group;
    const u32 zrows = two ? ((nb + 2 * key_group - 1) / (2 * key_group)) * key_group : nb;
    dim3 grid((N / 2 + TPB - 1) / TPB, L, zrows);
#define RME(M_, K_, R_, E_)                                                                                                            \
    hipLaunchKernelGGL((relin_mac_kernel<M_, K_, R_, E_>), grid, dim3(TPB), 0, st, dc, N, L, d01, stride01, dig, key, mask, out, out_map, \
                       key_stride, key_group, sigma_T, mask_div, nb, eqp, eqp_M)
#define RM(M_, K_, R_) RME(M_, K_, R_, false)
#define RQ(K_, R_) RME(true, K_, R_, true)
    if (eqp && two) {
        if (kp == 16) RQ(16, 2); else if (kp == 8) RQ(8, 2); else RQ(0, 2);
    } else if (eqp) {
        if (kp == 16) RQ(16, 1); else if (kp == 8) RQ(8, 1); else RQ(0, 1);
    } else if (two) {
        if (kp == 16) RM(true, 16, 2); else if (kp == 8) RM(true, 8, 2); else RM(true, 0, 2);
    } else if (small_moduli) {
        if (kp == 16) RM(true, 16, 1); else if (kp == 8) RM(true, 8, 1); else RM(true, 0, 1);
    } else {
        if (kp == 16) RM(false, 16, 1); else if (kp == 8) RM(false, 8, 1); else RM(false, 0, 1);
    }
#undef RQ
#undef RM
#undef RME
}

__global__ void host_flag_kernel(volatile u64 *flag, u64 value)
{
    *flag = value;
    __threadfence_system();
}
void launch_host_flag(u64 *flag_dev, u64 value, hipStream_t st)
{
    hipLaunchKernelGGL(host_flag_kernel, dim3(1), dim3(1), 0, st, (volatile u64 *)flag_dev, value);
}

__global__ void __launch_bounds__(TPB) ct_add_kernel(const DevConsts *dc, u32 N, u32 L, const u64 *__restrict__ x,
                                                     const u64 *__restrict__ y, u64 *__restrict__ out)
{
    const u32 n = blockIdx.x * TPB + threadIdx.x;
    if (n >= N) return;
    const u32 l = blockIdx.y % L;
    const size_t o = ((size_t)blockIdx.z * 2 * L + blockIdx.y) * N + n;
    out[o] = addmod(x[o], y[o], dc->mod[l].q);
}
void launch_ct_add(const DevConsts *dc, u32 N, u32 L, const u64 *x, const u64 *y, u64 *out, u32 nct, hipStream_t st)
{
    dim3 grid((N + TPB - 1) / TPB, 2 * L, nct);
    hipLaunchKernelGGL(ct_add_kernel, grid, dim3(TPB), 0, st, dc, N, L, x, y, out);
}
__global__ void __launch_bounds__(TPB) ct_mul_plain_kernel(const DevConsts *dc, u32 N, u32 L, const u64 *__restrict__ x,
                                                           const u64 *__restrict__ pt, size_t pt_stride,
                                                           u64 *__restrict__ out, u32 pt_div)
{
    const u32 n = blockIdx.x * TPB + threadIdx.x;
    if (n >= N) return;
    const u32 l = blockIdx.y % L;
    const size_t o = ((size_t)blockIdx.z * 2 * L + blockIdx.y) * N + n;
    out[o] = mulmod(x[o], pt[(size_t)(blockIdx.z / pt_div) * pt_stride + (size_t)l * N + n], dc->mod[l]);
}
void launch_ct_mul_plain(const DevConsts *dc, u32 N, u32 L, const u64 *x, const u64 *pt, size_t pt_stride, u64 *out,
                         u32 nct, hipStream_t st, u32 pt_div)
{
    dim3 grid((N + TPB - 1) / TPB, 2 * L, nct);
    hipLaunchKernelGGL(ct_mul_plain_kernel, grid, dim3(TPB), 0, st, dc, N, L, x, pt, pt_stride, out, pt_div ? pt_div : 1);
}

template <int L, int KEEP>
__global__ void __launch_bounds__(TPB) limb_drop_kernel(const DevConsts *__restrict__ dc, u32 N, u32 blocks_per_poly,
                                                        const u64 *__restrict__ in, u64 *__restrict__ out)
{
    const u32 poly = blockIdx.x / blocks_per_poly;
    const u32 n = (blockIdx.x % blocks_per_poly) * TPB + threadIdx.x;
    if (n >= N) return;
    const u64 *pin = in + (size_t)poly * L * N + n;
    u64 c[L];
#pragma unroll
    for (int i = 0; i < L; i++) c[i] = pin[(size_t)i * N];
#pragma unroll
    for (int l = L - 1; l >= KEEP; l--) {
        const u64 ql = dc->mod[l].q;
        const u64 v = c[l];
        const u64 s = (u64)((int64_t)((ql >> 1) - v) >> 63);
#pragma unroll
        for (int i = 0; i < l; i++) {
            const u64 off = dc->drop_off[l][i];
            const u64 x = c[i] - v + off + (s & (ql - off));
            c[i] = mul_shoup_u(x, dc->drop_inv[l][i], dc->drop_inv_sh[l][i], dc->mod[i].q, dc->drop_negq[i]);
        }
    }
    u64 *pout = out + (size_t)poly * KEEP * N + n;
#pragma unroll
    for (int i = 0; i < KEEP; i++) pout[(size_t)i * N] = c[i];
}
bool launch_limb_drop(const DevConsts *dc, u32 N, u32 L, u32 keep, const u64 *in, u64 *out, u32 npoly, hipStream_t st)
{
    if (keep < 1 || keep >= L || L > MAX_L || !npoly) return false;
    const u32 bpp = (N + TPB - 1) / TPB;
    const dim3 grid(bpp * npoly), block(TPB);
#define DROP_(L_, K_)                                                                                          \
    case (L_) * 8 + (K_):                                                                                      \
        hipLaunchKernelGGL((limb_drop_kernel<L_, K_>), grid, block, 0, st, dc, N, bpp, in, out);               \
        return true
    switch (L * 8 + keep) {
        DROP_(2, 1);
        DROP_(3, 1); DROP_(3, 2);
        DROP_(4, 1); DROP_(4, 2); DROP_(4, 3);
        DROP_(5, 1); DROP_(5, 2); DROP_(5, 3); DROP_(5, 4);
        DROP_(6, 1); DROP_(6, 2); DROP_(6, 3); DROP_(6, 4); DROP_(6, 5);
        DROP_(7, 1); DROP_(7, 2); DROP_(7, 3); DROP_(7, 4); DROP_(7, 5); DROP_(7, 6);
    }
#undef DROP_
    return false;
}

__global__ void __launch_bounds__(TPB) permute_kernel(u32 N, const u64 *__restrict__ in, const u32 *__restrict__ map,
                                                      u64 *__restrict__ out)
{
    const u32 p = blockIdx.x * TPB + threadIdx.x;
    if (p >= N) return;
    const size_t r = (size_t)blockIdx.y * N;
    out[r + p] = in[r + map[p]];
}
void launch_permute(u32 N, const u64 *in, const u32 *map, u64 *out, u32 nrows, hipStream_t st)
{
    dim3 grid((N + TPB - 1) / TPB, nrows);
    hipLaunchKernelGGL(permute_kernel, grid, dim3(TPB), 0, st, N, in, map, out);
}

__global__ void __launch_bounds__(TPB) bcast_mul_plain_kernel(const DevConsts *dc, u32 N, u32 L, const u64 *__restrict__ x,
                                                              size_t xs, u32 group, const u64 *__restrict__ pt, size_t ps_outer,
                                                              size_t ps_inner, u64 *__restrict__ out)
{
    const u32 n = blockIdx.x * TPB + threadIdx.x;
    if (n >= N) return;
    const u32 l = blockIdx.y % L, i = blockIdx.z, g = i / group, r = i % group;
    const size_t LN = (size_t)L * N;
    const size_t o = (size_t)blockIdx.y * N + n;
    out[(size_t)i * 2 * LN + o] = mulmod(x[(size_t)g * xs + o], pt[(size_t)g * ps_outer + (size_t)r * ps_inner + (size_t)l * N + n], dc->mod[l]);
}
void launch_bcast_mul_plain(const DevConsts *dc, u32 N, u32 L, const u64 *x, size_t xs, u32 group, const u64 *pt, size_t ps_outer,
                            size_t ps_inner, u64 *out, u32 nct, hipStream_t st)
{
    dim3 grid((N + TPB - 1) / TPB, 2 * L, nct);
    hipLaunchKernelGGL(bcast_mul_plain_kernel, grid, dim3(TPB), 0, st, dc, N, L, x, xs, group, pt, ps_outer, ps_inner, out);
}
__global__ void __launch_bounds__(TPB) rot_prepare_kernel(const DevConsts *dc, u32 N, u32 L, const u64 *__restrict__ x,
                                                          const u32 *__restrict__ maps, u32 map_group, u32 acc, u32 identity_first,
                                                          u64 *__restrict__ d01, u64 *__restrict__ d2)
{
    const u32 p = blockIdx.x * TPB + threadIdx.x;
    if (p >= N) return;
    const u32 l = blockIdx.y, i = blockIdx.z, r = i % map_group;
    const size_t LN = (size_t)L * N;
    const u64 *c0 = x + (size_t)i * 2 * LN + (size_t)l * N, *c1 = c0 + LN;
    u64 *o0 = d01 + (size_t)i * 2 * LN + (size_t)l * N, *o1 = o0 + LN, *o2 = d2 + (size_t)i * LN + (size_t)l * N;
    if (identity_first && r == 0) {
        o0[p] = c0[p];
        o1[p] = c1[p];
        o2[p] = 0;
        return;
    }
    const u32 s = maps[(size_t)r * N + p];
    const u64 q = dc->mod[l].q;
    o0[p] = acc ? addmod(c0[p], c0[s], q) : c0[s];
    o1[p] = acc ? c1[p] : 0;
    o2[p] = c1[s];
}
void launch_rot_prepare(const DevConsts *dc, u32 N, u32 L, const u64 *x, const u32 *maps, u32 map_group, bool acc, bool identity_first,
                        u64 *d01, u64 *d2, u32 nct, hipStream_t st)
{
    dim3 grid((N + TPB - 1) / TPB, L, nct);
    hipLaunchKernelGGL(rot_prepare_kernel, grid, dim3(TPB), 0, st, dc, N, L, x, maps, map_group ? map_group : 1u, acc ? 1u : 0u,
                       identity_first ? 1u : 0u, d01, d2);
}
__global__ void __launch_bounds__(TPB) sum_mul_plain_kernel(const DevConsts *dc, u32 N, u32 L, const u64 *__restrict__ x, u32 group,
                                                            const u64 *__restrict__ pt, size_t pt_stride, u64 *__restrict__ out,
                                                            size_t out_stride)
{
    const u32 n = blockIdx.x * TPB + threadIdx.x;
    if (n >= N) return;
    const u32 l = blockIdx.y % L, g = blockIdx.z;
    const size_t LN = (size_t)L * N;
    const size_t o = (size_t)blockIdx.y * N + n;
    const Mod m = dc->mod[l];
    u64 s = 0;
    for (u32 r = 0; r < group; r++) s = addmod(s, x[((size_t)g * group + r) * 2 * LN + o], m.q);
    out[(size_t)g * out_stride + o] = mulmod(s, pt[(size_t)g * pt_stride + (size_t)l * N + n], m);
}
void launch_sum_mul_plain(const DevConsts *dc, u32 N, u32 L, const u64 *x, u32 group, const u64 *pt, size_t pt_stride, u64 *out,
                          size_t out_stride, u32 ngroups, hipStream_t st)
{
    dim3 grid((N + TPB - 1) / TPB, 2 * L, ngroups);
    hipLaunchKernelGGL(sum_mul_plain_kernel, grid, dim3(TPB), 0, st, dc, N, L, x, group, pt, pt_stride, out, out_stride);
}

__global__ void __launch_bounds__(TPB) encode_scatter_kernel(const DevConsts *dc, u32 N, u32 M,
                                                             const int64_t *__restrict__ slots, u32 B,
                                                             const u32 *__restrict__ inv_pos, u64 *__restrict__ u)
{
    const u32 p = blockIdx.x * TPB + threadIdx.x;
    if (p >= N) return;
    const u64 t = dc->mod[M].q;
    const u32 s = inv_pos[p];
    u64 val = 0;
    if (s < B) {
        const int64_t v = slots[(size_t)blockIdx.y * B + s];
        const u64 mag = v < 0 ? (u64)(-v) : (u64)v;
        val = v < 0 ? (mag ? t - mag : 0) : mag;
    }
    u[(size_t)blockIdx.y * N + p] = val;
}
void launch_encode_scatter(const DevConsts *dc, u32 N, u32 M, const int64_t *slots, u32 B, const u32 *inv_pos, u64 *u,
                           u32 npt, hipStream_t st)
{
    dim3 grid((N + TPB - 1) / TPB, npt);
    hipLaunchKernelGGL(encode_scatter_kernel, grid, dim3(TPB), 0, st, dc, N, M, slots, B, inv_pos, u);
}
__global__ void __launch_bounds__(TPB) encode_lift_kernel(const DevConsts *dc, u32 N, u32 L, u32 M,
                                                          const u64 *__restrict__ u, u64 *__restrict__ out, u32 l0)
{
    const u32 n = blockIdx.x * TPB + threadIdx.x;
    if (n >= N) return;
    const u64 t = dc->mod[M].q;
    const u64 v = u[(size_t)blockIdx.z * N + n];
    const u64 q = dc->mod[l0 + blockIdx.y].q;
    out[((size_t)blockIdx.z * L + blockIdx.y) * N + n] = v > t / 2 ? q - (t - v) : v;
}
void launch_encode_lift(const DevConsts *dc, u32 N, u32 L, u32 M, const u64 *u, u64 *out, u32 npt, hipStream_t st, u32 l0)
{
    dim3 grid((N + TPB - 1) / TPB, L, npt);
    hipLaunchKernelGGL(encode_lift_kernel, grid, dim3(TPB), 0, st, dc, N, L, M, u, out, l0);
}

}
```

### nested_hashing_psi_amd/csrc/params.cpp

```cpp
#include "params.hpp"

#include <string.h>

namespace piehip {

typedef unsigned __int128 u128;

static inline u64 mm(u64 a, u64 b, u64 q) { return (u64)(((u128)a * b) % q); }

u64 powmod(u64 a, u64 e, u64 q)
{
    u64 r = 1 % q;
    a %= q;
    for (; e; e >>= 1) {
        if (e & 1) r = mm(r, a, q);
        a = mm(a, a, q);
    }
    return r;
}
u64 invmod(u64 a, u64 q) { return powmod(a % q, q - 2, q); }

u32 bitrev32(u32 x, u32 bits)
{
    u32 r = 0;
    for (u32 i = 0; i < bits; i++, x >>= 1) r = (r << 1) | (x & 1);
    return r;
}

bool is_prime_u64(u64 n)
{
    static const u64 B[] = {2, 3, 5, 7, 11, 13, 17, 19, 23, 29, 31, 37};
    if (n < 2) return false;
    for (u64 b : B) {
        if (n == b) return true;
        if (n % b == 0) return false;
    }
    u64 d = n - 1;
    int s = 0;
    for (; !(d & 1); d >>= 1) s++;
    for (u64 b : B) {
        u64 x = powmod(b, d, n);
        if (x == 1 || x == n - 1) continue;
        bool witness = true;
        for (int r = 1; r < s && witness; r++) {
            x = mm(x, x, n);
            if (x == n - 1) witness = false;
        }
        if (witness) return false;
    }
    return true;
}

bool prime_chain(u32 N, u64 below, u32 count, u64 *out)
{
    const u64 step = 2ULL * N;
    if (below <= step + 1) return false;
    u64 c = ((below - 2) / step) * step + 1;
    u32 got = 0;
    for (; got < count && c > step; c -= step)
        if (is_prime_u64(c)) out[got++] = c;
    return got == count;
}

u64 min_primitive_root(u64 q, u32 N)
{
    const u64 m = 2ULL * N;
    if ((q - 1) % m) return 0;
    u64 root = 0;
    for (u64 g = 2; g < 1000 && !root; g++) {
        u64 x = powmod(g, (q - 1) / m, q);
        if (powmod(x, N, q) == q - 1) root = x;
    }
    if (!root) return 0;
    const u64 sq = mm(root, root, q);
    u64 cur = root, best = root;
    for (u32 k = 1; k < N; k++) {
        cur = mm(cur, sq, q);
        if (cur < best) best = cur;
    }
    return best;
}

static inline u64 shoup(u64 w, u64 q) { return (u64)(((u128)w << 64) / q); }

static Mod make_mod(u64 q, u32 N)
{
    Mod m;
    memset(&m, 0, sizeof(m));
    m.q = q;
    u128 ratio = (~(u128)0) / q;
    m.r0 = (u64)ratio;
    m.r1 = (u64)(ratio >> 64);
    m.fshift = (u32)__builtin_clzll(q);
    m.fconst = (u64)((((u128)1) << (127 - m.fshift)) / q);
    m.n_inv = invmod(N, q);
    m.n_inv_sh = shoup(m.n_inv, q);
    return m;
}

static u64 prod_mod(const u64 *ms, u32 n, int skip, u64 q)
{
    u64 r = 1 % q;
    for (u32 k = 0; k < n; k++)
        if ((int)k != skip) r = mm(r, ms[k] % q, q);
    return r;
}

std::string HostParams::init(u32 N_, u32 L_, u64 t_, const u64 *q, const u64 *p)
{
    if (N_ < 8 || (N_ & (N_ - 1)) || N_ > (1u << 16)) return "N must be a power of two in [8, 65536]";
    if (L_ < 1 || L_ > MAX_L) return "L must be in [1, 7]";
    if ((t_ - 1) % (2ULL * N_) || !is_prime_u64(t_)) return "plaintext modulus t must be prime and = 1 (mod 2N)";
    N = N_;
    L = L_;
    M = 2 * L + 1;
    t = t_;
    logN = 0;
    while ((1u << logN) < N) logN++;
    moduli.assign(M + 1, 0);
    if (q && p) {
        for (u32 i = 0; i < L; i++) moduli[i] = q[i];
        for (u32 j = 0; j <= L; j++) moduli[L + j] = p[j];
    } else if (!q && !p) {
        if (!prime_chain(N, 1ULL << 60, M, moduli.data())) return "prime chain exhausted";
    } else {
        return "pass both q and p, or neither";
    }
    moduli[M] = t;
    for (u32 a = 0; a < M; a++) {
        const u64 m = moduli[a];
        if (m >> 61) return "RNS primes must be < 2^61";
        if (m <= t) return "RNS primes must exceed the plaintext modulus";
        if ((m - 1) % (2ULL * N) || !is_prime_u64(m)) return "RNS moduli must be prime and = 1 (mod 2N)";
        for (u32 b = 0; b < a; b++)
            if (moduli[b] == m) return "RNS moduli must be distinct";
    }

    psi.assign(M + 1, 0);
    tw.assign(M + 1, {});
    tw_sh.assign(M + 1, {});
    itw.assign(M + 1, {});
    itw_sh.assign(M + 1, {});
    memset(&dc, 0, sizeof(dc));
    dc.N = N;
    dc.logN = logN;
    dc.L = L;
    dc.M = M;
    for (u32 a = 0; a <= M; a++) {
        const u64 m = moduli[a];
        dc.mod[a] = make_mod(m, N);
        psi[a] = min_primitive_root(m, N);
        if (!psi[a]) return "no primitive 2N-th root";
        const u64 ipsi = invmod(psi[a], m);
        tw[a].assign(N, 0);
        itw[a].assign(N, 0);
        tw_sh[a].assign(N, 0);
        itw_sh[a].assign(N, 0);
        u64 pw = 1, ipw = 1;
        for (u32 e = 0; e < N; e++) {
            const u32 k = bitrev32(e, logN);
            tw[a][k] = pw;
            itw[a][k] = ipw;
            tw_sh[a][k] = shoup(pw, m);
            itw_sh[a][k] = shoup(ipw, m);
            pw = mm(pw, psi[a], m);
            ipw = mm(ipw, ipsi, m);
        }
        dc.fold_w[a] = tw[a][1];
        dc.fold_w_sh[a] = tw_sh[a][1];
        dc.fold_ia[a] = dc.mod[a].n_inv;
        dc.fold_ia_sh[a] = dc.mod[a].n_inv_sh;
        dc.fold_ib[a] = mm(itw[a][1], dc.mod[a].n_inv, m);
        dc.fold_ib_sh[a] = shoup(dc.fold_ib[a], m);
    }

    slot_pos.assign(N, 0);
    {
        const u64 m2 = 2ULL * N;
        u64 e = 1;
        for (u32 i = 0; i < N / 2; i++) {
            slot_pos[i] = bitrev32((u32)((e - 1) / 2), logN);
            slot_pos[N / 2 + i] = bitrev32((u32)((m2 - e - 1) / 2), logN);
            e = (e * 5) % m2;
        }
    }

    const u64 *Q = moduli.data();
    const u64 *P = moduli.data() + L;
    const u32 Lp = L + 1;
    for (u32 i = 0; i < L; i++) {
        const u64 qi = Q[i];
        dc.qhat_inv[i] = invmod(prod_mod(Q, L, (int)i, qi), qi);
        dc.qhat_inv_sh[i] = shoup(dc.qhat_inv[i], qi);
        dc.P_modq[i] = prod_mod(P, Lp, -1, qi);
        dc.P_modq_sh[i] = shoup(dc.P_modq[i], qi);
        dc.tPinv_modq[i] = mm(t % qi, invmod(dc.P_modq[i], qi), qi);
        dc.tPinv_modq_sh[i] = shoup(dc.tPinv_modq[i], qi);
        for (u32 j = 0; j < Lp; j++) {
            const u64 pj = P[j];
            dc.qhat_modp[i][j] = prod_mod(Q, L, (int)i, pj);
            const u64 v = mm(dc.P_modq[i] % pj, invmod(qi, pj), pj);
            dc.PI_modp[i][j] = v ? pj - v : 0;
        }
        for (u32 j = 0; j < L; j++) dc.qi_modqj[i][j] = qi % Q[j];
        dc.t_inv_modq[i] = invmod(t % qi, qi);
        dc.fold_iaq[i] = mm(dc.fold_ia[i], dc.qhat_inv[i], qi);
        dc.fold_iaq_sh[i] = shoup(dc.fold_iaq[i], qi);
        dc.fold_ibq[i] = mm(dc.fold_ib[i], dc.qhat_inv[i], qi);
        dc.fold_ibq_sh[i] = shoup(dc.fold_ibq[i], qi);
        dc.t_modq_sh[i] = shoup(t % qi, qi);
    }
    for (u32 j = 0; j < Lp; j++) {
        const u64 pj = P[j];
        dc.Q_modp[j] = prod_mod(Q, L, -1, pj);
        dc.phat_inv[j] = invmod(prod_mod(P, Lp, (int)j, pj), pj);
        dc.phat_inv_sh[j] = shoup(dc.phat_inv[j], pj);
        dc.tQ_modp[j] = mm(t % pj, dc.Q_modp[j], pj);
        dc.tQ_modp_sh[j] = shoup(dc.tQ_modp[j], pj);
        for (u32 i = 0; i < L; i++) {
            const u64 qi = Q[i];
            dc.phat_modq[j][i] = prod_mod(P, Lp, (int)j, qi);
            const u64 v = mm(dc.tQ_modp[j] % qi, invmod(pj, qi), qi);
            dc.tQF_modq[j][i] = v ? qi - v : 0;
        }
    }
    dc.Q_modt = prod_mod(Q, L, -1, t);
    for (u32 a = 0; a < M; a++) {
        dc.qp_hat_inv[a] = invmod(prod_mod(moduli.data(), M, (int)a, moduli[a]), moduli[a]);
        dc.qp_hat_inv_sh[a] = shoup(dc.qp_hat_inv[a], moduli[a]);
    }
    for (u32 j = 0; j < Lp; j++) {
        const u64 pj = P[j];
        dc.fold_iap[j] = mm(dc.fold_ia[L + j], dc.qp_hat_inv[L + j], pj);
        dc.fold_iap_sh[j] = shoup(dc.fold_iap[j], pj);
        dc.fold_ibp[j] = mm(dc.fold_ib[L + j], dc.qp_hat_inv[L + j], pj);
        dc.fold_ibp_sh[j] = shoup(dc.fold_ibp[j], pj);
    }
    for (u32 k = 0; k < L; k++) {
        const u64 qk = Q[k];
        dc.fold_iat[k] = mm(dc.fold_ia[k], dc.tPinv_modq[k], qk);
        dc.fold_iat_sh[k] = shoup(dc.fold_iat[k], qk);
        dc.fold_ibt[k] = mm(dc.fold_ib[k], dc.tPinv_modq[k], qk);
        dc.fold_ibt_sh[k] = shoup(dc.fold_ibt[k], qk);
    }
    for (u32 l = 0; l < L; l++) {
        const u64 half = (Q[l] - 1) / 2;
        dc.drop_negq[l] = 0 - Q[l];
        for (u32 i = 0; i < l; i++) {
            const u64 qi = Q[i];
            dc.drop_inv[l][i] = invmod(Q[l] % qi, qi);
            dc.drop_inv_sh[l][i] = shoup(dc.drop_inv[l][i], qi);
            dc.drop_off[l][i] = (half + qi - 1) / qi * qi;
        }
    }
    return "";
}

std::vector<u32> HostParams::automorph_map(u32 g) const
{
    std::vector<u32> map(N);
    const u64 m2 = 2ULL * N;
    for (u32 p = 0; p < N; p++) {
        const u64 e = ((2ULL * bitrev32(p, logN) + 1) * g) % m2;
        map[p] = bitrev32((u32)((e - 1) / 2), logN);
    }
    return map;
}

}
```

### nested_hashing_psi_amd/csrc/params.hpp

```cpp
#pragma once
#include <stdint.h>

#include <string>
#include <vector>

#include "modarith.h"

namespace piehip {

static const u32 MAX_L = 7;
static const u32 MAX_M = 2 * MAX_L + 1;

struct DevConsts {
    Mod mod[MAX_M + 1];
    u64 qhat_inv[8];
    u64 qhat_inv_sh[8];
    u64 qhat_modp[8][8];
    u64 Q_modp[8];
    u64 P_modq[8];
    u64 P_modq_sh[8];
    u64 PI_modp[8][8];
    u64 phat_inv[8];
    u64 phat_inv_sh[8];
    u64 phat_modq[8][8];
    u64 qp_hat_inv[16];
    u64 qp_hat_inv_sh[16];
    u64 tPinv_modq[8];
    u64 tPinv_modq_sh[8];
    u64 tQ_modp[8];
    u64 tQ_modp_sh[8];
    u64 tQF_modq[8][8];
    u64 qi_modqj[8][8];
    u64 fold_w[MAX_M + 1], fold_w_sh[MAX_M + 1];
    u64 fold_ia[MAX_M + 1], fold_ia_sh[MAX_M + 1];
    u64 fold_ib[MAX_M + 1], fold_ib_sh[MAX_M + 1];
    u64 fold_iaq[8], fold_iaq_sh[8], fold_ibq[8], fold_ibq_sh[8];
    u64 fold_iap[8], fold_iap_sh[8], fold_ibp[8], fold_ibp_sh[8];
    u64 fold_iat[8], fold_iat_sh[8], fold_ibt[8], fold_ibt_sh[8];
    u64 t_inv_modq[8];
    u64 t_modq_sh[8];
    u64 Q_modt;
    u64 drop_inv[8][8], drop_inv_sh[8][8];
    u64 drop_off[8][8];
    u64 drop_negq[8];
    u32 N, logN, L, M;
};

struct HostParams {
    u32 N = 0, logN = 0, L = 0, M = 0;
    u64 t = 0;
    std::vector<u64> moduli;
    std::vector<u64> psi;
    std::vector<std::vector<u64>> tw, tw_sh, itw, itw_sh;
    std::vector<u32> slot_pos;
    DevConsts dc;

    std::string init(u32 N, u32 L, u64 t, const u64 *q, const u64 *p);
    std::vector<u32> automorph_map(u32 g) const;
};

bool is_prime_u64(u64 n);
bool prime_chain(u32 N, u64 below, u32 count, u64 *out);
u64 min_primitive_root(u64 q, u32 N);
u64 powmod(u64 a, u64 e, u64 q);
u64 invmod(u64 a, u64 q);
u32 bitrev32(u32 x, u32 bits);

}
```

### nested_hashing_psi_amd/csrc/piehip_run.cpp

```cpp
#include <cassert>

#include "piehip_ctx.hpp"

using namespace piehip;

namespace piehip {

void ntt(piehip_ctx *h, u64 *data, u32 nlimbs, u32 mod_base, u32 mod_count, bool inv, bool sigma, bool fold, const NttExtra *ex)
{
    ProfScope ps(h, inv ? PIEHIP_K_NTT_INV : PIEHIP_K_NTT_FWD, 16.0 * h->hp.N * nlimbs);
    launch_ntt(h->plan, data, nlimbs, mod_base, mod_count, inv, h->stream, sigma && h->plan.lane_order, fold && h->plan.fold, ex);
}

void enqueue_keyswitch(piehip_ctx *h, MulWs &w, u32 nb, const u64 *key, const u64 *mask, u64 *out, bool lane, size_t key_stride,
                       u32 key_group, bool out_is_result, bool digits_ready, bool d01_eval_q)
{
    const NttPlan &pl = h->plan;
    const u32 N = h->hp.N, L = h->hp.L;
    const size_t LN = h->LN();
    const double W = 8.0 * N;
    lane = lane && pl.lane_order;
    if (digits_ready) {
    } else if (lane ? pl.digit_lift_lane : pl.digit_lift_std) {
        ProfScope ps(h, PIEHIP_K_NTT_FWD, 16.0 * N * nb * L * L);
        launch_ntt_digits(pl, w.d2c, w.dig, nb, L, lane, h->stream);
    } else {
        {
            ProfScope ps(h, PIEHIP_K_DIGITS, W * nb * (L + (double)L * L));
            launch_digits(h->d_dc, N, L, w.d2c, LN, nb, w.dig, h->stream, lane && pl.fold);
        }
        ntt(h, w.dig, nb * L * L, 0, L, false, lane, lane);
    }
    {
        if (h->wait_before_results && out_is_result) (void)hipStreamWaitEvent(h->stream, h->wait_before_results, 0);
        if (h->chain_armed && out_is_result) {
            h->chain_armed = false;
            (void)hipEventRecord(h->ev_chain, h->stream);
        }
        assert(!d01_eval_q || (pl.d01_eval_q && lane));
        ProfScope ps(h, PIEHIP_K_RELIN,
                     W * (nb * ((double)L * L + 2 * L + 2 * L + (mask ? L : 0) + (d01_eval_q ? 4 * L : 0)) + 2.0 * L * L));
        launch_relin_mac(h->d_dc, N, L, w.d01, 2 * LN, w.dig, key, mask, out, nb, h->stream, pl.small_moduli,
                         lane ? h->d_sigma_inv : nullptr, key_stride, key_group, lane ? pl.lane_T : 0, pl.lane_kp, mask ? h->mask_div : 1,
                         d01_eval_q ? w.eqp : nullptr, h->hp.M);
    }
}

struct RunKey {
    const u64 *key;
    size_t stride;
    u32 group;
};
static RunKey run_key(const piehip_ctx *h)
{
    const bool lane = h->plan.lane_order;
    if (h->key_group > 1) return {lane ? h->d_evkq_sigma : h->d_evkq, (size_t)h->hp.L * 2 * h->LN(), h->key_group};
    return {lane ? h->d_evk_sigma : h->d_evk, 0, 1};
}

void enqueue_mul(piehip_ctx *h, MulWs &w, const u64 *x, size_t sx, const u64 *y, size_t sy, u32 nb, bool relin,
                 const u64 *mask, u64 *out, bool xq_ready, bool out_is_result)
{
    const u32 N = h->hp.N, L = h->hp.L, M = h->hp.M;
    const size_t LN = h->LN();
    const double W = 8.0 * N;
    const NttPlan &pl = h->plan;
    {
        ProfScope ps(h, PIEHIP_K_EXPAND, W * nb * (4.0 * L + 4.0 * M));
        launch_expand_both(h->d_dc, N, L, x, sx, y, sy, LN, nb, w.eqp, h->stream, pl.small_moduli, pl.fold, xq_ready);
    }
    {
        NttExtra ex;
        ex.lazy_out = true;
        if (xq_ready) {
            ex.skip_L = L;
            ex.skip_M = M;
        }
        ntt(h, w.eqp, nb * (xq_ready ? 4 * M - 2 * L : 4 * M), 0, M, false, true, true, &ex);
    }
    const bool eval_q = relin && pl.d01_eval_q;
    if (pl.fused_tensor) {
        ProfScope ps(h, PIEHIP_K_TENSOR_NTT_INV, W * nb * 7.0 * M);
        launch_ntt16_tensor(pl, w.eqp, w.dqp, nb, M, h->stream, eval_q ? L : 0);
    } else {
        {
            ProfScope ps(h, PIEHIP_K_TENSOR, W * nb * 7.0 * M);
            launch_tensor(h->d_dc, N, M, w.eqp, w.dqp, nb, h->stream, pl.small_moduli);
        }
        ntt(h, w.dqp, nb * 3 * M, 0, M, true, true, true);
    }
    if (relin) {
        {
            ProfScope ps(h, PIEHIP_K_SCALE, W * nb * (3.0 * M + 3.0 * L));
            launch_scale_round(h->d_dc, N, L, w.dqp, nb, w.d01, 2 * LN, w.d2c, LN, h->stream, pl.small_moduli, pl.fold, false, eval_q);
        }
        NttExtra ex;
        ex.lazy_out = true;
        if (pl.digits_with_d01) {
            ProfScope ps(h, PIEHIP_K_NTT_FWD, 16.0 * N * nb * (2.0 * L + (double)L * L));
            Ntt16Digits dg = {w.d2c, LN, w.dig, nb, L};
            launch_ntt16(pl, w.d01, nb * 2 * L, 0, L, false, true, h->stream, &ex, &dg);
        } else {
            ntt(h, w.d01, nb * 2 * L, 0, L, false, true, true, &ex);
        }
        const RunKey k = run_key(h);
        enqueue_keyswitch(h, w, nb, k.key, mask, out, true, k.stride, k.group, out_is_result, pl.digits_with_d01, eval_q);
    } else {
        {
            ProfScope ps(h, PIEHIP_K_SCALE, W * nb * (3.0 * M + 3.0 * L));
            launch_scale_round(h->d_dc, N, L, w.dqp, nb, out, 3 * LN, out + 2 * LN, 3 * LN, h->stream, pl.small_moduli, pl.fold, true);
        }
        ntt(h, out, nb * 3 * L, 0, L, false, false, true);
    }
}

void enqueue_mod_reduce(piehip_ctx *h, u64 *full, u32 rows, u32 keep, u64 *out, bool out_is_result)
{
    const u32 N = h->hp.N, L = h->hp.L;
    const double W = 8.0 * N;
    {
        ProfScope ps(h, PIEHIP_K_RESULT_NTT_INV, 2 * W * rows * 2 * L);
        launch_ntt(h->plan, full, rows * 2 * L, 0, L, true, h->stream);
    }
    if (out_is_result) {
        if (h->wait_before_results) (void)hipStreamWaitEvent(h->stream, h->wait_before_results, 0);
        if (h->chain_armed) {
            h->chain_armed = false;
            (void)hipEventRecord(h->ev_chain, h->stream);
        }
    }
    {
        ProfScope ps(h, PIEHIP_K_LIMB_DROP, W * rows * 2 * (L + keep));
        launch_limb_drop(h->d_dc, N, L, keep, full, out, rows * 2, h->stream);
    }
    {
        ProfScope ps(h, PIEHIP_K_RESULT_NTT_FWD, 2 * W * rows * 2 * keep);
        launch_ntt(h->plan, out, rows * 2 * keep, 0, keep, false, h->stream);
    }
}

static const u32 MAX_RUN_QUEUES = 2;
u32 run_queue_count(const piehip_ctx *h)
{
    const u32 want = h->run_streams ? h->run_streams : (h->b >= 8 ? 2u : 1u);
    return std::min(want, std::min(MAX_RUN_QUEUES, h->b));
}

int ensure_run_queues(piehip_ctx *h, u32 ng)
{
    while (h->side_streams.size() < ng) {
        hipStream_t s = nullptr;
        hipEvent_t e = nullptr;
        HIPCHK(hipStreamCreateWithFlags(&s, hipStreamNonBlocking));
        h->side_streams.push_back(s);
        HIPCHK(hipEventCreateWithFlags(&e, hipEventDisableTiming));
        h->ev_join.push_back(e);
    }
    return PIEHIP_OK;
}

bool run_x_direct(const piehip_ctx *h) { return h->K > 1 && h->nq > 1 && h->plan.x_direct; }

u32 run_group_size(u32 b, u32 ng, u32 g)
{
    if (ng == 2) {
        const u32 first = (4 * b + 3) / 7;
        return g == 0 ? first : b - first;
    }
    return b / ng + (g < b % ng ? 1 : 0);
}

}

extern "C" {

static void enqueue_run_bins_full(piehip_ctx *h, u32 b0, u32 nb, u64 *results, bool chain_only);
static void enqueue_chain_bins(piehip_ctx *h, u32 b0, u32 layers, u64 *results);
static void enqueue_run_bins(piehip_ctx *h, u32 b0, u32 nb, u64 *results, bool chain_only)
{
    const u32 keep = h->res_limbs, nq = h->nq;
    if (keep >= h->hp.L) {
        enqueue_run_bins_full(h, b0, nb, results, chain_only);
        return;
    }
    const hipEvent_t wait = h->wait_before_results;
    const bool chain = h->chain_armed;
    h->wait_before_results = nullptr;
    h->chain_armed = false;
    enqueue_run_bins_full(h, b0, nb, h->d_full, chain_only);
    h->wait_before_results = wait;
    h->chain_armed = chain;
    const size_t r0 = (size_t)b0 * nq;
    enqueue_mod_reduce(h, h->d_full + r0 * 2 * h->LN(), nb * nq, keep, results + r0 * h->res_ct_words(), true);
}
static void enqueue_run_bins_full(piehip_ctx *h, u32 b0, u32 nb, u64 *results, bool chain_only)
{
    const u32 N = h->hp.N, L = h->hp.L, M = h->hp.M, K = h->K, b = h->b, E = h->E, nq = h->nq;
    const size_t LN = h->LN();
    const double W = 8.0 * N;
    const size_t r0 = (size_t)b0 * nq;
    const u32 layers = nb;
    nb *= nq;
    u64 *acc = h->d_acc + r0 * K * 2 * LN;
    const bool x_direct = run_x_direct(h);
    if (h->profiling) {
        ProfScope ps(h, PIEHIP_K_EVENT_PAIR, 0.0);
    }
    if (!chain_only) {
        ProfScope ps(h, PIEHIP_K_STAGE_A, W * ((double)layers * K * E * L + nq * ((double)K * E * 2 * L + 2.0 * L + (double)layers * K * 2 * L)));
        StageAQueries qs = {};
        for (u32 q = 0; q < nq; q++) qs.idx[q] = h->query[q].idx, qs.minus[q] = h->query[q].minus;
        const u64 *db = h->d_db + (size_t)b0 * E * LN;
        StageAXOut xo;
        if (x_direct) xo.out = h->ws.eqp + r0 * 4 * M * N, xo.M = M, xo.logns = h->plan.lane_logn;
        if (nq > 1) {
            launch_stage_a_batch(h->d_dc, N, L, K, layers, E, qs, nq, db, acc, h->stream, h->plan.small_moduli, b, 0, 0, x_direct ? &xo : nullptr);
        } else {
            launch_stage_a(h->d_dc, N, L, K, nb, E, qs.idx[0], qs.minus[0], db, acc, h->stream, h->plan.small_moduli, b, 0, 0, 1, 0,
                           x_direct ? &xo : nullptr);
        }
    }
    enqueue_chain_bins(h, b0, layers, results);
}
static void enqueue_chain_bins(piehip_ctx *h, u32 b0, u32 layers, u64 *results)
{
    const u32 N = h->hp.N, L = h->hp.L, M = h->hp.M, K = h->K, nq = h->nq;
    const size_t LN = h->LN();
    const double W = 8.0 * N;
    const size_t r0 = (size_t)b0 * nq;
    const u32 nb = layers * nq;
    MulWs w = h->ws;
    w.nb = nb;
    w.eqp += r0 * 4 * M * N;
    w.dqp += r0 * 3 * M * N;
    w.d01 += r0 * 2 * LN;
    w.d2c += r0 * LN;
    w.dig += r0 * L * LN;
    u64 *acc = h->d_acc + r0 * K * 2 * LN;
    u64 *prod = h->d_prod ? h->d_prod + r0 * 2 * LN : nullptr;
    u64 *out = results + r0 * 2 * LN;
    const u64 *masks = (h->plan.lane_order ? h->d_masks_sigma : h->d_masks) + (size_t)b0 * LN;
    struct MaskDiv {
        piehip_ctx *h;
        ~MaskDiv() { h->mask_div = h->key_group = 1; }
    } mask_div_scope{h};
    h->mask_div = nq;
    h->key_group = (nq > 1 && h->d_evkq && h->evkq_n == nq) ? nq : 1;
    const bool x_direct = run_x_direct(h);
    if (K == 1) {
        if (h->wait_before_results) (void)hipStreamWaitEvent(h->stream, h->wait_before_results, 0);
        ProfScope ps(h, PIEHIP_K_MASK, W * nb * 5.0 * L);
        launch_ct_mul_plain(h->d_dc, N, L, acc, h->d_masks + (size_t)b0 * LN, LN, out, nb, h->stream, nq);
        return;
    }
    const bool xq = h->plan.xq_reuse;
    NttExtra ex;
    ex.copy_out = w.eqp;
    ex.copy_K = K;
    ex.copy_L = L;
    ex.copy_M = M;
    ex.x_lane_in = x_direct;
    ntt(h, acc, nb * K * 2 * L, 0, L, true, false, true, xq ? &ex : nullptr);
    ex.x_lane_in = false;
    const u64 *x = acc;
    size_t sx = (size_t)K * 2 * LN;
    for (u32 hf = 1; hf < K; hf++) {
        const bool last = hf + 1 == K;
        u64 *dst = last ? out : prod;
        enqueue_mul(h, w, x, sx, acc + (size_t)hf * 2 * LN, (size_t)K * 2 * LN, nb, true, last ? masks : nullptr, dst, xq, last);
        if (!last) {
            ex.copy_K = 1;
            ntt(h, prod, nb * 2 * L, 0, L, true, false, true, xq ? &ex : nullptr);
            x = prod;
            sx = 2 * LN;
        }
    }
}

static hipError_t download_rows(piehip_ctx *h, const u64 *d_results, u32 b0, u32 nb)
{
    const size_t row = (size_t)h->nq * h->res_ct_words();
    return hipMemcpyAsync(h->host_results + (size_t)b0 * row, d_results + (size_t)b0 * row, (size_t)nb * row * sizeof(u64),
                          hipMemcpyDeviceToHost, h->stream);
}

}

int piehip::run_on_queues(piehip_ctx *h, void *d_results, bool chain_only)
{
    if (!h) return fail(PIEHIP_EINVAL, "null handle");
    if (!d_results) return fail(PIEHIP_EINVAL, "null result buffer");
    if (!chain_only && h->slice.on) return fail(PIEHIP_ESTATE, "run: a query-sliced handle holds no whole database (piehip_run_slice / piehip_run_chain)");
    if (!h->K || (!chain_only && !h->d_db)) return fail(PIEHIP_ESTATE, "run: database not loaded");
    if (!h->d_acc || !h->ws.eqp) return fail(PIEHIP_ESTATE, "run: no workspace (an earlier allocation failed: piehip_set_query_batch / load)");
    if (!run_keys_loaded(h)) return fail(PIEHIP_ESTATE, "run: relinearisation key not loaded");
    if (h->res_limbs < h->hp.L && !h->d_full) return fail(PIEHIP_ESTATE, "run: no rows for the result reduction (an earlier allocation failed: piehip_set_result_limbs)");
    for (u32 q = 0; q < h->nq && !chain_only; q++) {
        if (h->query[q].idx && h->query[q].minus) continue;
        if (q) return fail(PIEHIP_ESTATE, "run: a query of the batch has no index matrix or minus element");
        return fail(PIEHIP_ESTATE, "run: setIndex / setMinusCompareElement not called");
    }
    HIPCHK(hipSetDevice(h->device));
    const u32 b = h->b;
    h->recs.clear();
    h->pool_used = 0;
    const u32 ng = run_queue_count(h);
    if (ng > 1) {
        const int qrc = ensure_run_queues(h, ng);
        if (qrc) return qrc;
    }
    if (h->use_graph && !h->profiling && !h->host_results && h->nq == 1) {
        if (!h->gexec || h->g_idx != h->query[0].idx || h->g_minus != h->query[0].minus || h->g_res != d_results || h->g_ng != ng) {
            drop_graph(h);
            join_pending(h);
            struct Restore {
                piehip_ctx *h;
                hipStream_t s;
                ~Restore() { h->stream = s; }
            } restore{h, h->stream};
            hipGraph_t graph = nullptr;
            HIPCHK(hipStreamBeginCapture(restore.s, hipStreamCaptureModeThreadLocal));
            hipError_t ce = hipSuccess;
            if (ng > 1) {
                ce = hipEventRecord(h->ev_fork, restore.s);
                u32 b0 = 0;
                for (u32 g = 0; g < ng && ce == hipSuccess; g++) {
                    const u32 nb = run_group_size(b, ng, g);
                    ce = hipStreamWaitEvent(h->side_streams[g], h->ev_fork, 0);
                    h->stream = h->side_streams[g];
                    enqueue_run_bins(h, b0, nb, (u64 *)d_results, chain_only);
                    if (ce == hipSuccess) ce = hipEventRecord(h->ev_join[g], h->side_streams[g]);
                    if (ce == hipSuccess) ce = hipStreamWaitEvent(restore.s, h->ev_join[g], 0);
                    b0 += nb;
                }
                h->stream = restore.s;
            } else {
                enqueue_run_bins(h, 0, b, (u64 *)d_results, chain_only);
            }
            const hipError_t ee = hipStreamEndCapture(restore.s, &graph);
            if (ce != hipSuccess || ee != hipSuccess || !graph) {
                if (graph) (void)hipGraphDestroy(graph);
                return fail(PIEHIP_EHIP, std::string("run: graph capture failed: ") + hipGetErrorString(ce != hipSuccess ? ce : ee));
            }
            const hipError_t ie = hipGraphInstantiate(&h->gexec, graph, nullptr, nullptr, 0);
            (void)hipGraphDestroy(graph);
            if (ie != hipSuccess) {
                h->gexec = nullptr;
                return fail(PIEHIP_EHIP, std::string("run: hipGraphInstantiate: ") + hipGetErrorString(ie));
            }
            h->g_idx = h->query[0].idx, h->g_minus = h->query[0].minus, h->g_res = d_results, h->g_ng = ng;
        }
        join_pending(h);
        HIPCHK(hipGraphLaunch(h->gexec, h->stream));
        mark_dirty(h);
        return PIEHIP_OK;
    }
    if (ng > 1) {
        struct Restore {
            piehip_ctx *h;
            hipStream_t s;
            ~Restore()
            {
                h->stream = s;
                h->wait_before_results = nullptr;
            }
        } restore{h, h->stream};
        HIPCHK(hipEventRecord(h->ev_fork, restore.s));
        u32 b0 = 0;
        for (u32 g = 0; g < ng; g++) {
            const u32 nb = run_group_size(b, ng, g);
            if (h->inputs_dirty) HIPCHK(hipStreamWaitEvent(h->side_streams[g], h->ev_fork, 0));
            h->stream = h->side_streams[g];
            h->wait_before_results = h->inputs_dirty ? nullptr : h->ev_fork;
            if (h->host_results && g > 0) HIPCHK(hipStreamWaitEvent(h->side_streams[g], h->ev_chain, 0));
            if (h->host_results && g + 1 < ng) {
                if (!h->ev_chain) HIPCHK(hipEventCreateWithFlags(&h->ev_chain, hipEventDisableTiming));
                h->chain_armed = true;
            }
            enqueue_run_bins(h, b0, nb, (u64 *)d_results, chain_only);
            if (h->chain_armed) {
                h->chain_armed = false;
                HIPCHK(hipEventRecord(h->ev_chain, h->side_streams[g]));
            }
            if (h->host_results) HIPCHK(download_rows(h, (const u64 *)d_results, b0, nb));
            HIPCHK(hipEventRecord(h->ev_join[g], h->side_streams[g]));
            b0 += nb;
        }
        h->pending_join = true;
        h->inputs_dirty = false;
    } else {
        join_pending(h);
        enqueue_run_bins(h, 0, b, (u64 *)d_results, chain_only);
        if (h->host_results) HIPCHK(download_rows(h, (const u64 *)d_results, 0, b));
        mark_dirty(h);
    }
    HIPCHK(hipGetLastError());
    return PIEHIP_OK;
}

extern "C" {

int piehip_run_into(piehip_handle h, void *d_results) { return run_on_queues(h, d_results, false); }

int piehip_run(piehip_handle h)
{
    if (!h) return fail(PIEHIP_EINVAL, "null handle");
    if (!h->d_out) return fail(PIEHIP_ESTATE, "run: database not loaded");
    return piehip_run_into(h, h->d_out);
}

int piehip_join(piehip_handle h)
{
    NEED_RO(h);
    return PIEHIP_OK;
}

int piehip_set_graph(piehip_handle h, int on)
{
    NEED_RO(h);
    if (on && h->res_limbs < h->hp.L)
        return fail(PIEHIP_ESTATE, "set_graph: the captured graph hands out full results (piehip_set_result_limbs is below L)");
    if (on && h->slice.on) return fail(PIEHIP_ESTATE, "set_graph: a query-sliced handle runs in two halves (piehip_run_slice, piehip_run_chain): no captured graph");
    h->use_graph = on != 0;
    if (!on) drop_graph(h);
    return PIEHIP_OK;
}

int piehip_set_run_streams(piehip_handle h, uint32_t n)
{
    NEED_RO(h);
    h->run_streams = n;
    return PIEHIP_OK;
}

}
```

Before: 74490.

## Prescale y by t/P mod q during expansion to drop per-element Shoup multiplies

Folds the t·P^-1 mod q factor into the CRT constants used when expanding y into the QP basis (new phat_modq_y and P_modq_y tables). The later scale-round and relin MAC kernels can then skip their Shoup multiplications by tPinv on the Q-part of the evaluation-form data, and use unscaled fold twiddles. The eval-q accumulation block in relin_mac is also moved ahead of the key loop. Separately, the two-queue bin split ratio becomes a macro with default 8/14 instead of 4/7. The change adds template variants and DevConsts size, and correctness depends on the prescaled constants matching every consumer path.

```diff
diff --git a/nested_hashing_psi_amd/csrc/kernels.hpp b/nested_hashing_psi_amd/csrc/kernels.hpp
--- a/nested_hashing_psi_amd/csrc/kernels.hpp
+++ b/nested_hashing_psi_amd/csrc/kernels.hpp
@@ -48,6 +48,7 @@
     bool x_direct = false;
     bool fused_tensor = false;
     bool d01_eval_q = false;
+    bool y_prescaled = false;
     bool digits_with_d01 = false;
     bool digit_lift_lane = false;
     bool digit_lift_std = false;
@@ -91,6 +92,9 @@
 #ifndef PIEHIP_D01_EVAL_Q
 #define PIEHIP_D01_EVAL_Q 1
 #endif
+#ifndef PIEHIP_Y_PRESCALED
+#define PIEHIP_Y_PRESCALED 1
+#endif
 void launch_ntt16_tensor(const NttPlan &pl, const u64 *e, u64 *d, u32 nb, u32 M, hipStream_t st, u32 eval_q_L = 0);
 void launch_ntt_digits(const NttPlan &pl, const u64 *d2, u64 *dig, u32 nb, u32 L, bool sigma, hipStream_t st);
 
@@ -117,15 +121,17 @@
                             size_t in_stride_inner, u32 n_outer, u64 *out, u32 out_polys, u32 out_slot, hipStream_t st,
                             bool small_moduli, bool fold = false);
 void launch_expand_both(const DevConsts *dc, u32 N, u32 L, const u64 *x, size_t sx, const u64 *y, size_t sy, size_t si, u32 n_outer,
-                        u64 *out, hipStream_t st, bool small_moduli, bool fold = false, bool skip_q = false);
+                        u64 *out, hipStream_t st, bool small_moduli, bool fold = false, bool skip_q = false, bool y_prescaled = false);
 void launch_tensor(const DevConsts *dc, u32 N, u32 M, const u64 *e, u64 *d, u32 nb, hipStream_t st, bool small_moduli);
 void launch_scale_round(const DevConsts *dc, u32 N, u32 L, const u64 *d, u32 nb, u64 *out01, size_t stride01, u64 *out2,
-                        size_t stride2, hipStream_t st, bool small_moduli, bool fold = false, bool fold_comp2 = false, bool p_only01 = false);
+                        size_t stride2, hipStream_t st, bool small_moduli, bool fold = false, bool fold_comp2 = false, bool p_only01 = false,
+                        bool y_prescaled = false);
 void launch_digits(const DevConsts *dc, u32 N, u32 L, const u64 *d2, size_t stride2, u32 nb, u64 *dig, hipStream_t st,
                    bool fold = false);
 void launch_relin_mac(const DevConsts *dc, u32 N, u32 L, const u64 *d01, size_t stride01, const u64 *dig, const u64 *key,
                       const u64 *mask, u64 *out, u32 nb, hipStream_t st, bool small_moduli, const u32 *out_map = nullptr, size_t key_stride = 0,
-                      u32 key_group = 1, u32 sigma_T = 0, u32 sigma_kp = 16, u32 mask_div = 1, const u64 *eqp = nullptr, u32 eqp_M = 0);
+                      u32 key_group = 1, u32 sigma_T = 0, u32 sigma_kp = 16, u32 mask_div = 1, const u64 *eqp = nullptr, u32 eqp_M = 0,
+                      bool y_prescaled = false);
 void launch_bcast_mul_plain(const DevConsts *dc, u32 N, u32 L, const u64 *x, size_t xs, u32 group, const u64 *pt, size_t ps_outer,
                             size_t ps_inner, u64 *out, u32 nct, hipStream_t st);
 void launch_rot_prepare(const DevConsts *dc, u32 N, u32 L, const u64 *x, const u32 *maps, u32 map_group, bool acc, bool identity_first,
diff --git a/nested_hashing_psi_amd/csrc/kernels_ntt.hip b/nested_hashing_psi_amd/csrc/kernels_ntt.hip
--- a/nested_hashing_psi_amd/csrc/kernels_ntt.hip
+++ b/nested_hashing_psi_amd/csrc/kernels_ntt.hip
@@ -143,6 +143,7 @@
     pl.xq_reuse = ntt_route(pl, true, false, pl.fold).extra();
     pl.fused_tensor = PIEHIP_FUSE_TENSOR && k16 && small_moduli;
     pl.d01_eval_q = PIEHIP_D01_EVAL_Q && pl.fused_tensor;
+    pl.y_prescaled = PIEHIP_Y_PRESCALED && pl.d01_eval_q;
     pl.digits_with_d01 = k16 && small_moduli;
     pl.x_direct = pl.xq_reuse && k16 && small_moduli;
     const NttRoute std_fwd = ntt_route(pl, false, false, false);
diff --git a/nested_hashing_psi_amd/csrc/kernels_pie.hip b/nested_hashing_psi_amd/csrc/kernels_pie.hip
--- a/nested_hashing_psi_amd/csrc/kernels_pie.hip
+++ b/nested_hashing_psi_amd/csrc/kernels_pie.hip
@@ -585,7 +585,7 @@
     }
 }
 
-template <u32 L, bool MAD, bool YIN, int NP, bool LZ = false>
+template <u32 L, bool MAD, bool YIN, int NP, bool LZ = false, bool YS = false>
 __device__ __forceinline__ void scale_pq_core(const DevConsts *dc, const u64 (&x)[NP][L], u64 (&out)[NP][2 * L + 1])
 {
     constexpr u32 Lp = L + 1;
@@ -650,14 +650,14 @@
         const Mod mi = ld_mod(c, i);
         u64 hat[Lp];
 #pragma unroll
-        for (u32 j = 0; j < Lp; j++) hat[j] = c->phat_modq[j][i];
-        const u64 prodmod = c->P_modq[i], nq = neg_u(mi.q), n2q = neg_u(2 * mi.q);
+        for (u32 j = 0; j < Lp; j++) hat[j] = YS ? c->phat_modq_y[j][i] : c->phat_modq[j][i];
+        const u64 prodmod = YS ? c->P_modq_y[i] : c->P_modq[i], nq = neg_u(mi.q), n2q = neg_u(2 * mi.q);
 #pragma unroll
         for (int p = 0; p < NP; p++) out[p][i] = crt_out<Lp, MAD, LZ>(yp[p], hat, (fs2[p] + FIX_HALF) >> 60, prodmod, mi, nq, n2q);
     }
 }
 
-template <bool SCALE, bool FOLD, u32 L, bool MAD, bool SKIPQ>
+template <bool SCALE, bool FOLD, u32 L, bool MAD, bool SKIPQ, bool YS = false>
 __device__ __forceinline__ void expand_body(const DevConsts *__restrict__ dc, u32 N, const u64 *__restrict__ in, size_t so, size_t si,
                                             u64 *__restrict__ out, u32 out_polys, u32 out_slot, u32 by)
 {
@@ -687,7 +687,7 @@
     }
     constexpr bool LZ = FOLD && MAD;
     if (SCALE)
-        scale_pq_core<L, MAD, YIN, NP, LZ>(dc, x, y);
+        scale_pq_core<L, MAD, YIN, NP, LZ, YS>(dc, x, y);
     else
         expand_core<L, MAD, YIN, NP, LZ>(dc, x, y);
 #pragma unroll
@@ -711,31 +711,43 @@
 {
     expand_body<SCALE, FOLD, L, MAD, SKIPQ>(dc, N, in, so, si, out, out_polys, out_slot, blockIdx.y);
 }
-template <bool FOLD, u32 L, bool MAD, bool SKIPQ>
+template <bool FOLD, u32 L, bool MAD, bool SKIPQ, bool YS = false>
 __global__ void __launch_bounds__(TPB) expand_both_kernel(const DevConsts *__restrict__ dc, u32 N, const u64 *__restrict__ x, size_t sx,
                                                           const u64 *__restrict__ y, size_t sy, size_t si, u64 *__restrict__ out,
                                                           u32 n_outer)
 {
     if (blockIdx.y < 2 * n_outer)
-        expand_body<true, FOLD, L, MAD, false>(dc, N, y, sy, si, out, 4, 2, blockIdx.y);
+        expand_body<true, FOLD, L, MAD, false, YS>(dc, N, y, sy, si, out, 4, 2, blockIdx.y);
     else
         expand_body<false, FOLD, L, MAD, SKIPQ>(dc, N, x, sx, si, out, 4, 0, blockIdx.y - 2 * n_outer);
 }
 void launch_expand_both(const DevConsts *dc, u32 N, u32 L, const u64 *x, size_t sx, const u64 *y, size_t sy, size_t si, u32 n_outer,
-                        u64 *out, hipStream_t st, bool small_moduli, bool fold, bool skip_q)
-{
+                        u64 *out, hipStream_t st, bool small_moduli, bool fold, bool skip_q, bool y_prescaled)
+{
+    assert(!y_prescaled || (PIEHIP_Y_PRESCALED && small_moduli));
     dim3 grid(((fold ? N / 2 : N) + TPB - 1) / TPB, n_outer * 4);
-#define EB(F_, L_, M_, Q_) hipLaunchKernelGGL((expand_both_kernel<F_, L_, M_, Q_>), grid, dim3(TPB), 0, st, dc, N, x, sx, y, sy, si, out, n_outer)
+#define EBY(F_, L_, M_, Q_, Y_) \
+    hipLaunchKernelGGL((expand_both_kernel<F_, L_, M_, Q_, Y_>), grid, dim3(TPB), 0, st, dc, N, x, sx, y, sy, si, out, n_outer)
+#define EB(F_, L_, M_, Q_) EBY(F_, L_, M_, Q_, false)
+#if PIEHIP_Y_PRESCALED
+#define EBS(F_, L_, Q_) EBY(F_, L_, true, Q_, true)
+#else
+#define EBS(F_, L_, Q_) EB(F_, L_, true, Q_)
+#endif
 #define EBL(L_)                                                                          \
     case L_:                                                                             \
-        if (fold && small_moduli) { if (skip_q) EB(true, L_, true, true); else EB(true, L_, true, false); }      \
+        if (y_prescaled && fold) { if (skip_q) EBS(true, L_, true); else EBS(true, L_, false); }                  \
+        else if (y_prescaled) { if (skip_q) EBS(false, L_, true); else EBS(false, L_, false); }                   \
+        else if (fold && small_moduli) { if (skip_q) EB(true, L_, true, true); else EB(true, L_, true, false); }      \
         else if (fold) { if (skip_q) EB(true, L_, false, true); else EB(true, L_, false, false); }                 \
         else if (small_moduli) { if (skip_q) EB(false, L_, true, true); else EB(false, L_, true, false); }       \
         else { if (skip_q) EB(false, L_, false, true); else EB(false, L_, false, false); }                         \
         break;
     switch (L) { EBL(1) EBL(2) EBL(3) EBL(4) EBL(5) EBL(6) EBL(7) }
 #undef EBL
+#undef EBS
 #undef EB
+#undef EBY
 }
 
 static void launch_expand_common(bool scale, bool fold, const DevConsts *dc, u32 N, u32 L, const u64 *in, size_t so, size_t si,
@@ -830,7 +842,7 @@
         hipLaunchKernelGGL(tensor_kernel<false>, grid, dim3(TPB), 0, st, dc, N, M, e, d);
 }
 
-template <u32 L, bool MAD, int NP, bool PRE = false, bool PONLY = false>
+template <u32 L, bool MAD, int NP, bool PRE = false, bool PONLY = false, bool QPRE = false>
 __device__ __forceinline__ void scale_round_core(const DevConsts *dc, const u64 (&d)[NP][2 * L + 1], u64 (&out)[NP][L], bool lz = false)
 {
     constexpr u32 Lp = L + 1;
@@ -873,7 +885,7 @@
                 for (u32 j = 0; j < Lp; j++) colacc_mac(a, split30(yp[p][j]), split30(col[j]));
                 if (PONLY)
                     ;
-                else if (PRE)
+                else if (PRE || QPRE)
                     a.c0 += d[p][k];
                 else
                     colacc_mac(a, split30(d[p][k]), split30(tp));
@@ -882,7 +894,7 @@
                 U128 acc = dot128<Lp, MAD>(yp[p], col);
                 if (PONLY)
                     ;
-                else if (PRE)
+                else if (PRE || QPRE)
                     add128(acc, U128{d[p][k], 0});
                 else
                     mac128(acc, d[p][k], tp);
@@ -893,7 +905,7 @@
     }
 }
 
-template <bool FOLD, u32 L, bool MAD, bool PONLY>
+template <bool FOLD, u32 L, bool MAD, bool PONLY, bool QPRE = false>
 __device__ __forceinline__ void scale_round_comp(const DevConsts *__restrict__ dc, u32 N, u32 n, const u64 *__restrict__ pin,
                                                  u64 *__restrict__ pout, bool fold_out, bool lz)
 {
@@ -908,15 +920,17 @@
             const DcC c = dc_iter(dc);
             const u32 ak = a < L ? a : 0, aj = a < L ? 0 : a - L;
             const u64 q = c->mod[a].q, nq = neg_u(q), u = pin[(size_t)a * N], v = pin[(size_t)a * N + H];
-            const u64 wa = a < L ? c->fold_iat[ak] : c->fold_iap[aj], was = a < L ? c->fold_iat_sh[ak] : c->fold_iap_sh[aj];
-            const u64 wb = a < L ? c->fold_ibt[ak] : c->fold_ibp[aj], wbs = a < L ? c->fold_ibt_sh[ak] : c->fold_ibp_sh[aj];
+            const u64 wa = a >= L ? c->fold_iap[aj] : QPRE ? c->fold_ia[ak] : c->fold_iat[ak];
+            const u64 was = a >= L ? c->fold_iap_sh[aj] : QPRE ? c->fold_ia_sh[ak] : c->fold_iat_sh[ak];
+            const u64 wb = a >= L ? c->fold_ibp[aj] : QPRE ? c->fold_ib[ak] : c->fold_ibt[ak];
+            const u64 wbs = a >= L ? c->fold_ibp_sh[aj] : QPRE ? c->fold_ib_sh[ak] : c->fold_ibt_sh[ak];
             x[0][a] = shoup63(u + v, wa, was, nq);
             x[NP - 1][a] = shoup63(u + (4 * q - v), wb, wbs, nq);
         } else {
             x[0][a] = pin[(size_t)a * N];
         }
     }
-    scale_round_core<L, MAD, NP, FOLD, PONLY>(dc, x, y, lz);
+    scale_round_core<L, MAD, NP, FOLD, PONLY, QPRE>(dc, x, y, lz);
 #pragma unroll
     for (u32 k = 0; k < L; k++) {
         PIE_ITER_FENCE();
@@ -930,7 +944,7 @@
         }
     }
 }
-template <bool FOLD, u32 L, bool MAD, bool P01 = false>
+template <bool FOLD, u32 L, bool MAD, bool P01 = false, bool Q2PRE = false>
 __global__ void __launch_bounds__(TPB) scale_round_kernel(const DevConsts *__restrict__ dc, u32 N, const u64 *__restrict__ d,
                                                           u64 *__restrict__ out01, size_t stride01,
                                                           u64 *__restrict__ out2, size_t stride2, u32 fold_comp2)
@@ -945,15 +959,16 @@
     if (P01 && comp < 2)
         scale_round_comp<FOLD, L, MAD, true>(dc, N, n, pin, pout, true, lz);
     else
-        scale_round_comp<FOLD, L, MAD, false>(dc, N, n, pin, pout, comp < 2 || fold_comp2, lz);
+        scale_round_comp<FOLD, L, MAD, false, P01 && Q2PRE>(dc, N, n, pin, pout, comp < 2 || fold_comp2, lz);
 }
 void launch_scale_round(const DevConsts *dc, u32 N, u32 L, const u64 *d, u32 nb, u64 *out01, size_t stride01, u64 *out2,
-                        size_t stride2, hipStream_t st, bool small_moduli, bool fold, bool fold_comp2, bool p_only01)
+                        size_t stride2, hipStream_t st, bool small_moduli, bool fold, bool fold_comp2, bool p_only01, bool y_prescaled)
 {
     assert(!p_only01 || (small_moduli && !fold_comp2));
+    assert(y_prescaled == (p_only01 && PIEHIP_Y_PRESCALED));
     dim3 grid(((fold ? N / 2 : N) + TPB - 1) / TPB, 3, nb);
 #define SRK(F_, L_, M_, P_) \
-    hipLaunchKernelGGL((scale_round_kernel<F_, L_, M_, P_>), grid, dim3(TPB), 0, st, dc, N, d, out01, stride01, out2, stride2, (fold_comp2 && F_) ? 1u : 0u)
+    hipLaunchKernelGGL((scale_round_kernel<F_, L_, M_, P_, (P_) && PIEHIP_Y_PRESCALED>), grid, dim3(TPB), 0, st, dc, N, d, out01, stride01, out2, stride2, (fold_comp2 && F_) ? 1u : 0u)
 #define SRL(L_)                                                                        \
     case L_:                                                                           \
         if (p_only01) {                                                                \
@@ -1005,7 +1020,7 @@
         hipLaunchKernelGGL(digits_kernel<false>, grid, dim3(TPB), 0, st, dc, N, L, d2, stride2, dig);
 }
 
-template <bool MAD, int KP, int RPT = 1, bool EQ = false>
+template <bool MAD, int KP, int RPT = 1, bool EQ = false, bool YS = false>
 __global__ void __launch_bounds__(TPB) relin_mac_kernel(const DevConsts *__restrict__ dc, u32 N, u32 L, const u64 *__restrict__ d01,
                                                         size_t stride01, const u64 *__restrict__ dig,
                                                         const u64 *__restrict__ key0, const u64 *__restrict__ mask,
@@ -1050,6 +1065,34 @@
         for (int r = 0; r < RPT; r++)
 #pragma unroll
             for (int c = 0; c < 2; c++) a[r][c][0] = a[r][c][1] = ColAcc{0, 0, 0};
+        const u64 nq = 0 - m.q;
+        if (EQ) {
+            const u64 n2q = neg_u(2 * m.q), n4q = neg_u(4 * m.q);
+            u64 tp = 0, tpsh = 0;
+            if (!YS) tp = dc->tPinv_modq[j], tpsh = dc->tPinv_modq_sh[j];
+            const size_t MN = (size_t)eqp_M * N;
+#pragma unroll
+            for (int r = 0; r < RPT; r++) {
+                if (r && !has[r]) continue;
+                const u64 *pe = eqp + (size_t)rows[r] * 4 * MN + (size_t)j * N + n;
+                const u64x2 va0 = *reinterpret_cast<const u64x2 *>(pe), va1 = *reinterpret_cast<const u64x2 *>(pe + MN),
+                            vb0 = *reinterpret_cast<const u64x2 *>(pe + 2 * MN), vb1 = *reinterpret_cast<const u64x2 *>(pe + 3 * MN);
+#pragma unroll
+                for (int k = 0; k < 2; k++) {
+                    const Split30 sa0 = split30(csub_u(csub_u(k ? va0.y : va0.x, n4q), n2q)), sa1 = split30(csub_u(csub_u(k ? va1.y : va1.x, n4q), n2q));
+                    const Split30 sb0 = split30(csub_u(csub_u(k ? vb0.y : vb0.x, n4q), n2q)), sb1 = split30(csub_u(csub_u(k ? vb1.y : vb1.x, n4q), n2q));
+                    ColAcc t = {0, 0, 0};
+                    colacc_mac(t, sa0, sb0);
+                    const u64 r0 = colacc_reduce123_lazy(t, m, nq), v0 = YS ? r0 : shoup63_lazy(r0, tp, tpsh, nq);
+                    t = ColAcc{0, 0, 0};
+                    colacc_mac(t, sa0, sb1);
+                    colacc_mac(t, sa1, sb0);
+                    const u64 r1 = colacc_reduce123_lazy(t, m, nq), v1 = YS ? r1 : shoup63_lazy(r1, tp, tpsh, nq);
+                    a[r][0][k].c0 += v0 & 0x3FFFFFFFull, a[r][0][k].c1 += v0 >> 30;
+                    a[r][1][k].c0 += v1 & 0x3FFFFFFFull, a[r][1][k].c1 += v1 >> 30;
+                }
+            }
+        }
         for (u32 i = 0; i < L; i++) {
             const u64x2 k0 = *reinterpret_cast<const u64x2 *>(key + (((size_t)i * 2 + 0) * L + j) * N + n);
             const u64x2 k1 = *reinterpret_cast<const u64x2 *>(key + (((size_t)i * 2 + 1) * L + j) * N + n);
@@ -1063,33 +1106,6 @@
                 colacc_mac(a[r][0][1], dy, k0y);
                 colacc_mac(a[r][1][0], dx, k1x);
                 colacc_mac(a[r][1][1], dy, k1y);
-            }
-        }
-        const u64 nq = 0 - m.q;
-        if (EQ) {
-            const u64 n2q = neg_u(2 * m.q), n4q = neg_u(4 * m.q);
-            const u64 tp = dc->tPinv_modq[j], tpsh = dc->tPinv_modq_sh[j];
-            const size_t MN = (size_t)eqp_M * N;
-#pragma unroll
-            for (int r = 0; r < RPT; r++) {
-                if (r && !has[r]) continue;
-                const u64 *pe = eqp + (size_t)rows[r] * 4 * MN + (size_t)j * N + n;
-                const u64x2 va0 = *reinterpret_cast<const u64x2 *>(pe), va1 = *reinterpret_cast<const u64x2 *>(pe + MN),
-                            vb0 = *reinterpret_cast<const u64x2 *>(pe + 2 * MN), vb1 = *reinterpret_cast<const u64x2 *>(pe + 3 * MN);
-#pragma unroll
-                for (int k = 0; k < 2; k++) {
-                    const Split30 sa0 = split30(csub_u(csub_u(k ? va0.y : va0.x, n4q), n2q)), sa1 = split30(csub_u(csub_u(k ? va1.y : va1.x, n4q), n2q));
-                    const Split30 sb0 = split30(csub_u(csub_u(k ? vb0.y : vb0.x, n4q), n2q)), sb1 = split30(csub_u(csub_u(k ? vb1.y : vb1.x, n4q), n2q));
-                    ColAcc t = {0, 0, 0};
-                    colacc_mac(t, sa0, sb0);
-                    const u64 v0 = shoup63_lazy(colacc_reduce123_lazy(t, m, nq), tp, tpsh, nq);
-                    t = ColAcc{0, 0, 0};
-                    colacc_mac(t, sa0, sb1);
-                    colacc_mac(t, sa1, sb0);
-                    const u64 v1 = shoup63_lazy(colacc_reduce123_lazy(t, m, nq), tp, tpsh, nq);
-                    a[r][0][k].c0 += v0 & 0x3FFFFFFFull, a[r][0][k].c1 += v0 >> 30;
-                    a[r][1][k].c0 += v1 & 0x3FFFFFFFull, a[r][1][k].c1 += v1 >> 30;
-                }
             }
         }
 #pragma unroll
@@ -1167,9 +1183,10 @@
 }
 void launch_relin_mac(const DevConsts *dc, u32 N, u32 L, const u64 *d01, size_t stride01, const u64 *dig, const u64 *key,
                       const u64 *mask, u64 *out, u32 nb, hipStream_t st, bool small_moduli, const u32 *out_map, size_t key_stride,
-                      u32 key_group, u32 sigma_T, u32 sigma_kp, u32 mask_div, const u64 *eqp, u32 eqp_M)
+                      u32 key_group, u32 sigma_T, u32 sigma_kp, u32 mask_div, const u64 *eqp, u32 eqp_M, bool y_prescaled)
 {
     assert(!eqp || (small_moduli && eqp_M >= L));
+    assert(y_prescaled == (eqp != nullptr && PIEHIP_Y_PRESCALED));
     if (!key_group) key_group = 1;
     if (!mask_div) mask_div = 1;
     const bool tile = out_map && (sigma_kp == 16 || sigma_kp == 8) && sigma_T >= TPB / sigma_kp && sigma_T % (TPB / sigma_kp) == 0 &&
@@ -1179,7 +1196,7 @@
     const u32 zrows = two ? ((nb + 2 * key_group - 1) / (2 * key_group)) * key_group : nb;
     dim3 grid((N / 2 + TPB - 1) / TPB, L, zrows);
 #define RME(M_, K_, R_, E_)                                                                                                            \
-    hipLaunchKernelGGL((relin_mac_kernel<M_, K_, R_, E_>), grid, dim3(TPB), 0, st, dc, N, L, d01, stride01, dig, key, mask, out, out_map, \
+    hipLaunchKernelGGL((relin_mac_kernel<M_, K_, R_, E_, (E_) && PIEHIP_Y_PRESCALED>), grid, dim3(TPB), 0, st, dc, N, L, d01, stride01, dig, key, mask, out, out_map, \
                        key_stride, key_group, sigma_T, mask_div, nb, eqp, eqp_M)
 #define RM(M_, K_, R_) RME(M_, K_, R_, false)
 #define RQ(K_, R_) RME(true, K_, R_, true)
diff --git a/nested_hashing_psi_amd/csrc/params.cpp b/nested_hashing_psi_amd/csrc/params.cpp
--- a/nested_hashing_psi_amd/csrc/params.cpp
+++ b/nested_hashing_psi_amd/csrc/params.cpp
@@ -196,6 +196,7 @@
         dc.P_modq_sh[i] = shoup(dc.P_modq[i], qi);
         dc.tPinv_modq[i] = mm(t % qi, invmod(dc.P_modq[i], qi), qi);
         dc.tPinv_modq_sh[i] = shoup(dc.tPinv_modq[i], qi);
+        dc.P_modq_y[i] = mm(dc.tPinv_modq[i], dc.P_modq[i], qi);
         for (u32 j = 0; j < Lp; j++) {
             const u64 pj = P[j];
             dc.qhat_modp[i][j] = prod_mod(Q, L, (int)i, pj);
@@ -220,6 +221,7 @@
         for (u32 i = 0; i < L; i++) {
             const u64 qi = Q[i];
             dc.phat_modq[j][i] = prod_mod(P, Lp, (int)j, qi);
+            dc.phat_modq_y[j][i] = mm(dc.tPinv_modq[i], dc.phat_modq[j][i], qi);
             const u64 v = mm(dc.tQ_modp[j] % qi, invmod(pj, qi), qi);
             dc.tQF_modq[j][i] = v ? qi - v : 0;
         }
diff --git a/nested_hashing_psi_amd/csrc/params.hpp b/nested_hashing_psi_amd/csrc/params.hpp
--- a/nested_hashing_psi_amd/csrc/params.hpp
+++ b/nested_hashing_psi_amd/csrc/params.hpp
@@ -27,6 +27,8 @@
     u64 qp_hat_inv_sh[16];
     u64 tPinv_modq[8];
     u64 tPinv_modq_sh[8];
+    u64 phat_modq_y[8][8];
+    u64 P_modq_y[8];
     u64 tQ_modp[8];
     u64 tQ_modp_sh[8];
     u64 tQF_modq[8][8];
diff --git a/nested_hashing_psi_amd/csrc/piehip_run.cpp b/nested_hashing_psi_amd/csrc/piehip_run.cpp
--- a/nested_hashing_psi_amd/csrc/piehip_run.cpp
+++ b/nested_hashing_psi_amd/csrc/piehip_run.cpp
@@ -42,7 +42,7 @@
                      W * (nb * ((double)L * L + 2 * L + 2 * L + (mask ? L : 0) + (d01_eval_q ? 4 * L : 0)) + 2.0 * L * L));
         launch_relin_mac(h->d_dc, N, L, w.d01, 2 * LN, w.dig, key, mask, out, nb, h->stream, pl.small_moduli,
                          lane ? h->d_sigma_inv : nullptr, key_stride, key_group, lane ? pl.lane_T : 0, pl.lane_kp, mask ? h->mask_div : 1,
-                         d01_eval_q ? w.eqp : nullptr, h->hp.M);
+                         d01_eval_q ? w.eqp : nullptr, h->hp.M, d01_eval_q && pl.y_prescaled);
     }
 }
 
@@ -65,9 +65,10 @@
     const size_t LN = h->LN();
     const double W = 8.0 * N;
     const NttPlan &pl = h->plan;
+    const bool eval_q = relin && pl.d01_eval_q, y_pre = relin && pl.y_prescaled;
     {
         ProfScope ps(h, PIEHIP_K_EXPAND, W * nb * (4.0 * L + 4.0 * M));
-        launch_expand_both(h->d_dc, N, L, x, sx, y, sy, LN, nb, w.eqp, h->stream, pl.small_moduli, pl.fold, xq_ready);
+        launch_expand_both(h->d_dc, N, L, x, sx, y, sy, LN, nb, w.eqp, h->stream, pl.small_moduli, pl.fold, xq_ready, y_pre);
     }
     {
         NttExtra ex;
@@ -78,7 +79,6 @@
         }
         ntt(h, w.eqp, nb * (xq_ready ? 4 * M - 2 * L : 4 * M), 0, M, false, true, true, &ex);
     }
-    const bool eval_q = relin && pl.d01_eval_q;
     if (pl.fused_tensor) {
         ProfScope ps(h, PIEHIP_K_TENSOR_NTT_INV, W * nb * 7.0 * M);
         launch_ntt16_tensor(pl, w.eqp, w.dqp, nb, M, h->stream, eval_q ? L : 0);
@@ -92,7 +92,7 @@
     if (relin) {
         {
             ProfScope ps(h, PIEHIP_K_SCALE, W * nb * (3.0 * M + 3.0 * L));
-            launch_scale_round(h->d_dc, N, L, w.dqp, nb, w.d01, 2 * LN, w.d2c, LN, h->stream, pl.small_moduli, pl.fold, false, eval_q);
+            launch_scale_round(h->d_dc, N, L, w.dqp, nb, w.d01, 2 * LN, w.d2c, LN, h->stream, pl.small_moduli, pl.fold, false, eval_q, y_pre);
         }
         NttExtra ex;
         ex.lazy_out = true;
@@ -161,10 +161,13 @@
 
 bool run_x_direct(const piehip_ctx *h) { return h->K > 1 && h->nq > 1 && h->plan.x_direct; }
 
+#ifndef PIEHIP_RUN_FIRST_OF_14
+#define PIEHIP_RUN_FIRST_OF_14 8
+#endif
 u32 run_group_size(u32 b, u32 ng, u32 g)
 {
     if (ng == 2) {
-        const u32 first = (4 * b + 3) / 7;
+        const u32 first = (PIEHIP_RUN_FIRST_OF_14 * b + 7) / 14;
         return g == 0 ? first : b - first;
     }
     return b / ng + (g < b % ng ? 1 : 0);
```

New measurement: 74970 (median of 6 runs). Within noise of the previous version (+0.6%).
